# Schindler-EPFL-Lab/thermo-nerf

Hardware: AMD Instinct MI355X
Metric: rays/sec (forward-only render) @ 800x800, 192 samples/ray (higher is better)
Workload: dtype f32; 1 GPU; BASELINE metric configuration (configs[2]'s 192 samples/ray on the 800x800 frame of configs[1]): synthetic 800x800 RGB+thermal scene, P=(256,96)+192 samples/ray, chunk 640000, forward-only eval, scene weights; parallelism=ray-shard x1 (one frame per rank)

## Files before the change

### include/thermonerf_hip.h

```cpp
#ifndef THERMONERF_HIP_H
#define THERMONERF_HIP_H

#include <stddef.h>
#include <stdint.h>

#ifdef __cplusplus
extern "C" {
#endif

#define TN_OK 0
#define TN_ERR_NULL (-1)
#define TN_ERR_SHAPE (-2)
#define TN_ERR_UNSUPPORTED (-3)
#define TN_ERR_WORKSPACE (-4)
#define TN_ERR_LAUNCH (-5)

#define TN_MAX_LEVELS 16

typedef struct tn_hashgrid {
    const float *table;
    float scalings[TN_MAX_LEVELS];
    int32_t num_levels;
    int32_t log2_hashmap_size;
    const float *dense;
// ... 106 lines not shown
    float box_min[3], box_max[3];
    float thermal_lo, thermal_hi;
    float temperature_span, temperature_min;
    float to_world[12];
} tn_pointcloud_params;
int32_t tn_pointcloud_tile_rays(void);
int32_t tn_pointcloud_scan_width(void);
size_t tn_pointcloud_workspace_bytes(int64_t num_rays);
int tn_pointcloud_append(const float *origins, const float *directions, const float *depth, const float *accumulation,
                         const float *rgb, const float *thermal, int64_t num_rays, int64_t source_base,
                         const tn_pointcloud_params *params, const uint8_t *thermal_table, float *positions, uint8_t *colors,
                         float *temperature, uint8_t *thermal_colors, int64_t *source, int64_t capacity, int64_t *count,
                         void *workspace, size_t workspace_bytes, void *stream);

int32_t tn_knn_grid_resolution(int64_t num_points);
size_t tn_knn_workspace_bytes(int64_t num_points, int32_t grid_resolution);
int tn_knn(const float *positions, int64_t num_points, int32_t k, int32_t grid_resolution, int32_t *neighbor_index,
           float *neighbor_d2, double *mean_distance, void *workspace, size_t workspace_bytes, void *stream);
int tn_pointcloud_normals(const float *positions, const int32_t *neighbor_index, int64_t num_points, int32_t k,
                          const float *viewpoints, float *normals, void *stream);

typedef struct tn_mesh_params {
    float fx, fy, cx, cy;
    float w2c[12];
    float truncation, inv_truncation, min_accumulation;
    float lo[3], step[3];
    int32_t dims[3];
    float temperature_span, temperature_min;
    float to_world[12];
} tn_mesh_params;
int32_t tn_mesh_tile(void);
int32_t tn_mesh_scan_width(void);
size_t tn_mesh_workspace_bytes(int32_t nx, int32_t ny, int32_t nz);
int tn_tsdf_integrate(const float *depth, const float *accumulation, const float *thermal, const float *rgb, int32_t height,
                      int32_t width, const tn_mesh_params *params, float *volume, void *stream);
int tn_mesh_extract(const float *volume, const tn_mesh_params *params, const uint8_t *thermal_table, float *positions,
                    uint8_t *colors, float *temperature, uint8_t *thermal_colors, int64_t capacity_vertices, int32_t *triangles,
                    int64_t capacity_triangles, int64_t *counts, void *workspace, size_t workspace_bytes, void *stream);

size_t tn_mesh_components_workspace_bytes(int64_t num_vertices, int64_t num_triangles);
int tn_mesh_components(const int32_t *triangles, int64_t num_triangles, int64_t num_vertices, int32_t *labels,
                       int32_t *component_triangles, int64_t *summary, void *stream);
int tn_mesh_filter_components(const int32_t *triangles, int64_t num_triangles, int64_t num_vertices, const int32_t *labels,
                              const int32_t *component_triangles, const int64_t *summary, int64_t min_triangles,
                              int32_t largest_only, int32_t *vertex_source, int64_t capacity_vertices, int32_t *triangles_out,
                              int64_t capacity_triangles, int64_t *counts, void *workspace, size_t workspace_bytes, void *stream);

size_t tn_mesh_incidence_workspace_bytes(int64_t num_vertices, int64_t num_triangles);
int tn_mesh_incidence(const int32_t *triangles, int64_t num_triangles, int64_t num_vertices, int32_t *offsets, int32_t *corners,
                      void *workspace, size_t workspace_bytes, void *stream);
int tn_mesh_vertex_normals(const float *positions, const int32_t *triangles, int64_t num_triangles, int64_t num_vertices,
                           const int32_t *offsets, const int32_t *corners, float *normals, void *stream);
int tn_mesh_smooth(const float *positions_in, const int32_t *triangles, int64_t num_triangles, int64_t num_vertices,
                   const int32_t *offsets, const int32_t *corners, int32_t iterations, float lambda, float mu, float *positions_out,
                   float *scratch, void *stream);

int32_t tn_sort_tile(void);
size_t tn_sort_pairs_workspace_bytes(int64_t n);
int tn_sort_pairs(const uint64_t *keys_in, const int32_t *values_in, int64_t n, int key_bits, uint64_t *keys_out,
                  int32_t *values_out, void *workspace, size_t workspace_bytes, void *stream);

typedef struct tn_voxel_params {
    float origin[3];
    float voxel_size;
    int32_t dims[3];
} tn_voxel_params;
size_t tn_voxel_downsample_workspace_bytes(int64_t num_points);
int tn_voxel_downsample(const float *positions, const uint8_t *colors, const float *temperature, const uint8_t *thermal_colors,
                        const int64_t *source, int64_t num_points, const tn_voxel_params *params, float *positions_out,
                        uint8_t *colors_out, float *temperature_out, uint8_t *thermal_colors_out, int64_t *source_out,
                        int32_t *voxel_count, int64_t capacity, int64_t *count, void *workspace, size_t workspace_bytes, void *stream);


typedef struct tn_render_config {
    int32_t num_proposal_samples[2];
    int32_t num_nerf_samples;
    int32_t training;
    float pdf_anneal;
    float early_stop_transmittance;
    int32_t kernel_family;
    int32_t initial_sampler;
    int32_t sample_split;
    int32_t per_sample_jitter;
} tn_render_config;

typedef struct tn_render_inputs {
    const float *origins;
    const float *directions;
    const float *nears;
    const float *fars;
    const int32_t *camera_indices;
    const float *lin_bins0;
    const float *u1;
    const float *u2;
    const float *jitter;
} tn_render_inputs;

typedef struct tn_render_outputs {
    float *rgb;
    float *accumulation;
    float *depth;
    float *expected_depth;
    float *prop_depth_0;
    float *prop_depth_1;
    float *thermal;
    float *weights[3];
    float *spacing_bins[3];
    float *eucl_bins[3];
} tn_render_outputs;

size_t tn_render_workspace_bytes(const tn_render_config *cfg, int64_t num_rays);

int tn_render_rays_fwd(const tn_density_field *prop0, const tn_density_field *prop1, const tn_thermal_field *field,
                       const tn_render_config *cfg, const tn_render_inputs *in, const tn_render_outputs *out,
                       int64_t num_rays, void *workspace, size_t workspace_bytes, void *stream);

int tn_proposal_sample_fwd(const tn_density_field *prop0, const tn_density_field *prop1, const tn_render_config *cfg,
                           const tn_render_inputs *in, const tn_render_outputs *out, int64_t num_rays, void *workspace,
                           size_t workspace_bytes, void *stream);
int tn_field_render_fwd(const tn_thermal_field *field, const tn_render_config *cfg, const tn_render_inputs *in,
                        const tn_render_outputs *out, int64_t num_rays, void *workspace, size_t workspace_bytes,
                        void *stream);

int64_t tn_depth_bound_slots(int64_t first_ray, int64_t num_rays, int64_t chunk_rays);

int32_t tn_render_kernel_form(const tn_thermal_field *field, const tn_render_config *cfg, int64_t num_rays, int32_t pass);
int32_t tn_render_sample_split(const tn_thermal_field *field, const tn_render_config *cfg, int64_t num_rays);
int tn_field_render_chunked_fwd(const tn_thermal_field *field, const tn_render_config *cfg, const tn_render_inputs *in,
                                const tn_render_outputs *out, int64_t num_rays, void *workspace, size_t workspace_bytes,
                                int64_t first_ray, int64_t chunk_rays, float *depth_bounds, int32_t clip, void *stream);
int tn_expected_depth_clip_chunked(float *expected_depth, int64_t num_rays, int64_t first_ray, int64_t chunk_rays,
                                   const float *depth_bounds, void *stream);


size_t tn_hashgrid_prepare_bytes(const tn_hashgrid *grid, int64_t max_bytes);
int tn_hashgrid_prepare(const tn_hashgrid *grid_in, tn_hashgrid *grid_out, void *dense_dev, size_t dense_bytes,
                        void *stream);

size_t tn_field_prepare_bytes(const tn_thermal_field *field);
int tn_field_prepare(const tn_thermal_field *field, void *prepared_dev, size_t bytes, void *stream);

size_t tn_field_prepare_f16x3_bytes(const tn_thermal_field *field);
int tn_field_prepare_f16x3(const tn_thermal_field *field, void *prepared_dev, size_t bytes, void *stream);
size_t tn_field_prepare_bf16x6_bytes(const tn_thermal_field *field);
int tn_field_prepare_bf16x6(const tn_thermal_field *field, void *prepared_dev, size_t bytes, void *stream);

int tn_bf16x6_split_product(const float *a, const float *b, int64_t n, float *pieces_a, float *pieces_b, float *out, void *stream);
int tn_bf16_mfma_value_probe(float a_value, float b_value, float *out, void *stream);


#define TN_ACT_NONE 0
#define TN_ACT_RELU 1
#define TN_ACT_SIGMOID 2

int tn_hash_encode_fwd(const tn_hashgrid *grid, const tn_space *space, const float *positions, int64_t n, float *enc,
                       float *selector, void *stream);
int tn_hash_encode_bwd(const tn_hashgrid *grid, const tn_space *space, const float *positions, const float *d_enc,
                       int64_t n, float *d_table, void *stream);

int tn_hash_encode_bwd_levels(const tn_hashgrid *grid, const tn_space *space, const float *positions, const float *d_enc,
                              int64_t n, float *d_table, int32_t level_begin, int32_t level_end, void *stream);
size_t tn_hash_encode_bwd_spread_workspace_bytes(const tn_hashgrid *grid);
int tn_hash_encode_bwd_spread(const tn_hashgrid *grid, const tn_space *space, const float *positions, const float *d_enc,
                              int64_t n, float *d_table, int32_t level_begin, int32_t level_end, void *workspace,
                              size_t workspace_bytes, void *stream);

size_t tn_hash_encode_bwd_sorted_workspace_bytes(const tn_hashgrid *grid, int64_t n, int32_t level_begin);
int tn_hash_encode_bwd_sorted_first_level(const tn_hashgrid *grid, int64_t n);
int tn_hash_encode_bwd_sorted(const tn_hashgrid *grid, const tn_space *space, const float *positions, const float *d_enc,
                              int64_t n, float *d_table, int32_t level_begin, void *workspace, size_t workspace_bytes,
                              void *stream);

int tn_hash_encode_bwd_input(const tn_hashgrid *grid, const tn_space *space, const float *positions, const float *d_enc,
                             int64_t n, float *d_positions, void *stream);
int tn_frustum_positions_bwd(const float *d_positions, const float *starts, const float *ends, int64_t num_rays, int32_t n,
                             float *d_origins, float *d_directions, void *stream);

int tn_linear_fwd(const float *x, int32_t ldx, const tn_linear *lin, int32_t act, int64_t n, float *y, int32_t ldy,
                  void *stream);
size_t tn_linear_bwd_workspace_bytes(void);
int tn_linear_bwd(const float *x, int32_t ldx, const float *y, const float *dy, int32_t ldy, const tn_linear *lin,
                  int32_t act, int64_t n, float *dx, int32_t lddx, int32_t accumulate_dx, float *d_weight,
                  float *d_bias, void *workspace, size_t workspace_bytes, void *stream);

int tn_density_act_fwd(const float *raw, int32_t ld_raw, const float *selector, float average_init_density, int64_t n,
                       float *density, void *stream);
int tn_density_act_bwd(const float *raw, int32_t ld_raw, const float *selector, float average_init_density,
                       float trunc_exp_min, const float *d_density, int64_t n, float *d_raw, int32_t ld_d_raw,
                       int32_t clear_cols, void *stream);

int tn_weights_bwd(const float *deltas, const float *densities, const float *d_weights, int64_t num_rays, int32_t n,
                   float *d_densities, void *stream);

typedef struct tn_chain_layer {
    tn_linear lin;
    const float *x;
    int32_t ldx;
    int32_t act_x;
    float *d_weight;
    float *d_bias;
} tn_chain_layer;
size_t tn_linear_chain_bwd_workspace_bytes(void);
int tn_linear_chain_bwd(const tn_chain_layer *layers, int32_t num_layers, const float *y_top, int32_t act_top, const float *dy,
                        int32_t lddy, int64_t n, float *dx, int32_t lddx, int32_t accumulate_dx, void *workspace,
                        size_t workspace_bytes, void *stream);

int tn_field_fwd_taped(const tn_thermal_field *field, const float *positions, const float *directions,
                       const int32_t *camera_indices, int64_t num_rays, int32_t n, float *enc, float *selector, float *h1,
                       float *bo, float *density, float *c1, float *c2, float *rgb, float *t1, float *t2, float *thermal,
                       void *stream);
// ... 152 lines not shown
```

### thermo_nerf_amd/_hip.py

```python
from __future__ import annotations

import ctypes as C
import os
from typing import Optional

import torch

_LIB_NAME = "libthermonerf_hip.so"
_LIB_PATH = os.environ.get("THERMONERF_HIP_LIB") or os.path.join(os.path.dirname(os.path.abspath(__file__)), _LIB_NAME)

TN_MAX_LEVELS = 16

TN_OK = 0
_ERRORS = {
    -1: "TN_ERR_NULL: a required pointer is NULL",
    -2: "TN_ERR_SHAPE: a dimension is out of the supported range",
    -3: "TN_ERR_UNSUPPORTED: configuration not implemented by the kernels",
    -4: "TN_ERR_WORKSPACE: workspace too small",
    -5: "TN_ERR_LAUNCH: HIP reported a launch error",
}

_f32p = C.POINTER(C.c_float)
_i32p = C.POINTER(C.c_int32)

# ... 27 lines not shown
                ("one_minus_beta2", C.c_float), ("eps", C.c_float), ("weight_decay", C.c_float)]


ADAM_MAX_TENSORS = 32

class tn_field_grads(C.Structure):
    _fields_ = [(k, C.c_void_p) for k in ("base0_w", "base0_b", "base1_w", "base1_b", "head0_w", "head1_w", "head1_b", "head2_w",
                                         "head2_b", "th0_w", "th0_b", "th1_w", "th1_b", "thead_w", "thead_b")]


class tn_space(C.Structure):
    _fields_ = [
        ("contraction", C.c_int32),
        ("aabb_min", C.c_float * 3),
        ("aabb_max", C.c_float * 3),
        ("_pad", C.c_int32),
    ]


class tn_pointcloud_params(C.Structure):
    _fields_ = [("min_accumulation", C.c_float), ("box_min", C.c_float * 3), ("box_max", C.c_float * 3), ("thermal_lo", C.c_float),
                ("thermal_hi", C.c_float), ("temperature_span", C.c_float), ("temperature_min", C.c_float),
                ("to_world", C.c_float * 12)]


class tn_voxel_params(C.Structure):
    _fields_ = [("origin", C.c_float * 3), ("voxel_size", C.c_float), ("dims", C.c_int32 * 3)]


class tn_mesh_params(C.Structure):
    _fields_ = [("fx", C.c_float), ("fy", C.c_float), ("cx", C.c_float), ("cy", C.c_float), ("w2c", C.c_float * 12),
                ("truncation", C.c_float), ("inv_truncation", C.c_float), ("min_accumulation", C.c_float), ("lo", C.c_float * 3),
                ("step", C.c_float * 3), ("dims", C.c_int32 * 3), ("temperature_span", C.c_float), ("temperature_min", C.c_float),
                ("to_world", C.c_float * 12)]


class tn_density_field(C.Structure):
    _fields_ = [
        ("grid", tn_hashgrid),
        ("l0", tn_linear),
        ("l1", tn_linear),
        ("space", tn_space),
        ("average_init_density", C.c_float),
        ("_pad", C.c_int32),
    ]


class tn_thermal_field(C.Structure):
    _fields_ = [
        ("grid", tn_hashgrid),
        ("base0", tn_linear),
        ("base1", tn_linear),
        ("head0", tn_linear),
        ("head1", tn_linear),
        ("head2", tn_linear),
        ("th0", tn_linear),
        ("th1", tn_linear),
        ("thead", tn_linear),
        ("appearance", C.c_void_p),
        ("num_images", C.c_int32),
        ("app_dim", C.c_int32),
        ("geo_feat_dim", C.c_int32),
        ("use_average_appearance", C.c_int32),
        ("sh_shifted", C.c_int32),
        ("space", tn_space),
        ("average_init_density", C.c_float),
        ("prepared", C.c_void_p),
        ("prepared_f16x3", C.c_void_p),
        ("prepared_bf16x6", C.c_void_p),
    ]


class tn_render_config(C.Structure):
    _fields_ = [
        ("num_proposal_samples", C.c_int32 * 2),
        ("num_nerf_samples", C.c_int32),
        ("training", C.c_int32),
        ("pdf_anneal", C.c_float),
        ("early_stop_transmittance", C.c_float),
        ("kernel_family", C.c_int32),
        ("initial_sampler", C.c_int32),
        ("sample_split", C.c_int32),
        ("per_sample_jitter", C.c_int32),
    ]


class tn_render_inputs(C.Structure):
    _fields_ = [
        ("origins", C.c_void_p),
        ("directions", C.c_void_p),
        ("nears", C.c_void_p),
        ("fars", C.c_void_p),
        ("camera_indices", C.c_void_p),
        ("lin_bins0", C.c_void_p),
        ("u1", C.c_void_p),
        ("u2", C.c_void_p),
        ("jitter", C.c_void_p),
    ]


class tn_render_outputs(C.Structure):
    _fields_ = [
        ("rgb", C.c_void_p),
        ("accumulation", C.c_void_p),
        ("depth", C.c_void_p),
        ("expected_depth", C.c_void_p),
        ("prop_depth_0", C.c_void_p),
        ("prop_depth_1", C.c_void_p),
        ("thermal", C.c_void_p),
        ("weights", C.c_void_p * 3),
        ("spacing_bins", C.c_void_p * 3),
        ("eucl_bins", C.c_void_p * 3),
    ]


_fp = C.c_void_p


class tn_train_step(C.Structure):
    _fields_ = [("prop0", C.POINTER(tn_density_field)), ("prop1", C.POINTER(tn_density_field)),
                ("field_raw", C.POINTER(tn_thermal_field)), ("field", C.POINTER(tn_thermal_field)), ("prepared_bytes", C.c_size_t),
                ("cfg", C.POINTER(tn_render_config)), ("inputs", C.POINTER(tn_render_inputs)), ("num_rays", C.c_int64),
                ("spacing", _fp * 3), ("eucl", _fp * 3), ("weights", _fp * 3), ("prop_depth", _fp * 2),
                ("positions", _fp), ("starts", _fp), ("ends", _fp), ("deltas", _fp), ("ray_bias", _fp),
                ("enc", _fp), ("selector", _fp), ("density", _fp), ("rgb_samples", _fp), ("thermal_samples", _fp), ("base_out", _fp),
                ("jacobian", _fp),
                ("rgb", _fp), ("thermal", _fp), ("accumulation", _fp), ("depth", _fp), ("expected_depth", _fp), ("depth_scratch", _fp),
                ("workspace", _fp), ("workspace_bytes", C.c_size_t), ("zero_buffer", _fp), ("zero_bytes", C.c_size_t),
                ("distortion_mult", C.c_float), ("interlevel_mult", C.c_float),
                ("distortion_loss_pair", _fp), ("distortion_grad", _fp), ("interlevel_loss", _fp), ("interlevel_grad", _fp * 2),
                ("stream", _fp), ("second", _fp), ("third", _fp), ("wait_events", C.POINTER(C.c_void_p)), ("num_wait_events", C.c_int32)]


class tn_train_step_bwd_args(C.Structure):
    _fields_ = [("field", C.POINTER(tn_thermal_field)), ("num_rays", C.c_int64), ("n", C.c_int32)] + [
        (k, _fp) for k in ("positions", "starts", "ends", "deltas", "ray_bias", "enc", "selector", "density", "rgb_samples",
                           "thermal_samples", "base_out", "jacobian", "accumulation", "directions", "camera_indices",
                           "d_rgb", "d_thermal", "d_accumulation", "d_weights")] + [
        ("use_gradient_scaling", C.c_int32), ("pass_thermal_gradients", C.c_int32), ("split_form", C.c_int32),
        ("sh_direction_gradient", C.c_int32), ("trunc_exp_min", C.c_float)] + [
        (k, _fp) for k in ("d_rgb_samples", "d_thermal_samples", "d_density", "d_enc", "d_positions", "d_ray_sum", "d_ray_inputs")] + [
        ("grads", C.POINTER(tn_field_grads)), ("d_table", _fp), ("d_appearance", _fp), ("d_head0_bias", _fp), ("d_origins", _fp),
        ("d_directions", _fp), ("fused_workspace", _fp), ("fused_workspace_bytes", C.c_size_t), ("first_sorted_level", C.c_int32),
        ("sorted_workspace", _fp), ("sorted_workspace_bytes", C.c_size_t), ("spread", C.c_int32), ("spread_workspace", _fp),
        ("spread_workspace_bytes", C.c_size_t), ("overlap", C.c_int32), ("defer", C.c_int32), ("wait_second_first", C.c_int32),
        ("stream", _fp), ("second", _fp), ("third", _fp)]


_vp, _i64, _i32, _sz = C.c_void_p, C.c_int64, C.c_int32, C.c_size_t
SIGNATURES = {
    "tn_generate_rays": (C.c_int, [C.POINTER(C.c_float), C.c_float, C.c_float, C.c_float, C.c_float, _i32, _i32,
                                   C.POINTER(C.c_float), _i64, _i64, _vp, _vp, _vp, _vp]),
    "tn_frustum_positions": (C.c_int, [_vp, _vp, _vp, _vp, _i64, _i32, _vp, _vp]),
    "tn_frustum_from_edges": (C.c_int, [_vp, _vp, _vp, _i64, _i32, _vp, _vp, _vp, _vp, _vp]),
    "tn_density_fwd": (C.c_int, [C.POINTER(tn_density_field), _vp, _i64, _vp, _vp]),
    "tn_field_density_fwd": (C.c_int, [C.POINTER(tn_thermal_field), _vp, _i64, _vp, _vp, _vp]),
    "tn_field_heads_fwd": (C.c_int, [C.POINTER(tn_thermal_field), _vp, _vp, _vp, _i64, _i32, _vp, _vp, _vp]),
    "tn_camera_opt_fwd": (C.c_int, [_vp, _vp, _vp, _vp, _i64, _i32, _vp, _vp, _vp]),
    "tn_camera_opt_bwd": (C.c_int, [_vp, _vp, _vp, _vp, _vp, _i64, _i32, _vp, _vp, _vp]),
    "tn_sample_initial": (C.c_int, [_vp, _vp, _vp, _vp, _i64, _i32, _i32, _vp, _vp, _vp]),
    "tn_weights_fwd": (C.c_int, [_vp, _vp, _i64, _i32, _vp, _vp]),
    "tn_sample_pdf": (C.c_int, [_vp, _vp, _vp, _vp, _vp, _vp, _i64, _i32, _i32, _i32, _vp, _vp, _vp]),
    "tn_composite_fwd": (C.c_int, [_vp, _vp, _i64, _i32, _i32, _i32, _vp, _vp]),
    "tn_depth_fwd": (C.c_int, [_vp, _vp, _vp, _i64, _i32, _vp, _vp, _vp, _vp, _vp]),
    "tn_ssim_workspace_bytes": (_sz, [_i32, _i32, _i32]),
    "tn_ssim_fwd": (C.c_int, [_vp, _vp, _i32, _i32, _i32, C.c_float, _vp, _sz, _vp, _vp]),
    "tn_frame_to_rgb8": (C.c_int, [_vp, _i64, _i32, _i32, _vp, _vp, _vp, _vp, _vp]),
    "tn_otsu_thresholds": (C.c_int, [_vp, C.POINTER(C.c_int64), _i32, _vp, _vp, _vp]),
    "tn_pointcloud_tile_rays": (_i32, []),
    "tn_pointcloud_scan_width": (_i32, []),
    "tn_pointcloud_workspace_bytes": (_sz, [_i64]),
    "tn_pointcloud_append": (C.c_int, [_vp] * 6 + [_i64, _i64, C.POINTER(tn_pointcloud_params)] + [_vp] * 6 + [_i64, _vp, _vp, _sz, _vp]),
    "tn_knn_grid_resolution": (_i32, [_i64]),
    "tn_knn_workspace_bytes": (_sz, [_i64, _i32]),
    "tn_knn": (C.c_int, [_vp, _i64, _i32, _i32, _vp, _vp, _vp, _vp, _sz, _vp]),
    "tn_pointcloud_normals": (C.c_int, [_vp, _vp, _i64, _i32, _vp, _vp, _vp]),
    "tn_sort_tile": (_i32, []),
    "tn_sort_pairs_workspace_bytes": (_sz, [_i64]),
    "tn_sort_pairs": (C.c_int, [_vp, _vp, _i64, C.c_int, _vp, _vp, _vp, _sz, _vp]),
    "tn_voxel_downsample_workspace_bytes": (_sz, [_i64]),
    "tn_voxel_downsample": (C.c_int, [_vp] * 5 + [_i64, C.POINTER(tn_voxel_params)] + [_vp] * 6 + [_i64, _vp, _vp, _sz, _vp]),
    "tn_mesh_tile": (_i32, []),
    "tn_mesh_scan_width": (_i32, []),
    "tn_mesh_workspace_bytes": (_sz, [_i32, _i32, _i32]),
    "tn_tsdf_integrate": (C.c_int, [_vp] * 4 + [_i32, _i32, C.POINTER(tn_mesh_params), _vp, _vp]),
    "tn_mesh_extract": (C.c_int, [_vp, C.POINTER(tn_mesh_params)] + [_vp] * 5 + [_i64, _vp, _i64, _vp, _vp, _sz, _vp]),
    "tn_mesh_components_workspace_bytes": (_sz, [_i64, _i64]),
    "tn_mesh_components": (C.c_int, [_vp, _i64, _i64, _vp, _vp, _vp, _vp]),
    "tn_mesh_filter_components": (C.c_int, [_vp, _i64, _i64, _vp, _vp, _vp, _i64, _i32, _vp, _i64, _vp, _i64, _vp, _vp, _sz, _vp]),
    "tn_mesh_incidence_workspace_bytes": (_sz, [_i64, _i64]),
    "tn_mesh_incidence": (C.c_int, [_vp, _i64, _i64, _vp, _vp, _vp, _sz, _vp]),
    "tn_mesh_vertex_normals": (C.c_int, [_vp, _vp, _i64, _i64, _vp, _vp, _vp, _vp]),
    "tn_mesh_smooth": (C.c_int, [_vp, _vp, _i64, _i64, _vp, _vp, _i32, C.c_float, C.c_float, _vp, _vp, _vp]),
    "tn_render_workspace_bytes": (_sz, [C.POINTER(tn_render_config), _i64]),
    "tn_render_rays_fwd": (
        C.c_int,
        [C.POINTER(tn_density_field), C.POINTER(tn_density_field), C.POINTER(tn_thermal_field),
         C.POINTER(tn_render_config), C.POINTER(tn_render_inputs), C.POINTER(tn_render_outputs), _i64, _vp, _sz, _vp],
    ),
    "tn_proposal_sample_fwd": (
        C.c_int,
        [C.POINTER(tn_density_field), C.POINTER(tn_density_field), C.POINTER(tn_render_config),
         C.POINTER(tn_render_inputs), C.POINTER(tn_render_outputs), _i64, _vp, _sz, _vp],
    ),
    "tn_field_render_fwd": (
        C.c_int,
        [C.POINTER(tn_thermal_field), C.POINTER(tn_render_config), C.POINTER(tn_render_inputs),
         C.POINTER(tn_render_outputs), _i64, _vp, _sz, _vp],
    ),
    "tn_bf16x6_split_product": (C.c_int, [_vp, _vp, _i64, _vp, _vp, _vp, _vp]),
    "tn_bf16_mfma_value_probe": (C.c_int, [C.c_float, C.c_float, _vp, _vp]),
    "tn_depth_bound_slots": (_i64, [_i64, _i64, _i64]),
    "tn_render_kernel_form": (C.c_int32, [C.POINTER(tn_thermal_field), C.POINTER(tn_render_config), _i64, C.c_int32]),
    "tn_render_sample_split": (C.c_int32, [C.POINTER(tn_thermal_field), C.POINTER(tn_render_config), _i64]),
    "tn_field_render_chunked_fwd": (
        C.c_int,
        [C.POINTER(tn_thermal_field), C.POINTER(tn_render_config), C.POINTER(tn_render_inputs),
         C.POINTER(tn_render_outputs), _i64, _vp, _sz, _i64, _i64, _vp, _i32, _vp],
    ),
    "tn_expected_depth_clip_chunked": (C.c_int, [_vp, _i64, _i64, _i64, _vp, _vp]),
    "tn_hashgrid_prepare_bytes": (_sz, [C.POINTER(tn_hashgrid), _i64]),
    "tn_hashgrid_prepare": (C.c_int, [C.POINTER(tn_hashgrid), C.POINTER(tn_hashgrid), _vp, _sz, _vp]),
    "tn_field_prepare_bytes": (_sz, [C.POINTER(tn_thermal_field)]),
    "tn_field_prepare": (C.c_int, [C.POINTER(tn_thermal_field), _vp, _sz, _vp]),
    "tn_field_prepare_f16x3_bytes": (_sz, [C.POINTER(tn_thermal_field)]),
    "tn_field_prepare_f16x3": (C.c_int, [C.POINTER(tn_thermal_field), _vp, _sz, _vp]),
    "tn_field_prepare_bf16x6_bytes": (_sz, [C.POINTER(tn_thermal_field)]),
    "tn_field_prepare_bf16x6": (C.c_int, [C.POINTER(tn_thermal_field), _vp, _sz, _vp]),
    "tn_hash_encode_fwd": (C.c_int, [C.POINTER(tn_hashgrid), C.POINTER(tn_space), _vp, _i64, _vp, _vp, _vp]),
    "tn_hash_encode_bwd": (C.c_int, [C.POINTER(tn_hashgrid), C.POINTER(tn_space), _vp, _vp, _i64, _vp, _vp]),
    "tn_hash_encode_bwd_levels": (C.c_int, [C.POINTER(tn_hashgrid), C.POINTER(tn_space), _vp, _vp, _i64, _vp, _i32, _i32, _vp]),
    "tn_hash_encode_bwd_spread_workspace_bytes": (_sz, [C.POINTER(tn_hashgrid)]),
    "tn_hash_encode_bwd_spread": (C.c_int, [C.POINTER(tn_hashgrid), C.POINTER(tn_space), _vp, _vp, _i64, _vp, _i32, _i32, _vp, _sz, _vp]),
    "tn_hash_encode_bwd_sorted_workspace_bytes": (_sz, [C.POINTER(tn_hashgrid), _i64, _i32]),
    "tn_hash_encode_bwd_sorted_first_level": (C.c_int, [C.POINTER(tn_hashgrid), _i64]),
    "tn_hash_encode_bwd_sorted": (C.c_int, [C.POINTER(tn_hashgrid), C.POINTER(tn_space), _vp, _vp, _i64, _vp, _i32, _vp, _sz, _vp]),
    "tn_linear_fwd": (C.c_int, [_vp, _i32, C.POINTER(tn_linear), _i32, _i64, _vp, _i32, _vp]),
    "tn_linear_bwd_workspace_bytes": (_sz, []),
    "tn_linear_bwd": (C.c_int, [_vp, _i32, _vp, _vp, _i32, C.POINTER(tn_linear), _i32, _i64, _vp, _i32, _i32, _vp, _vp, _vp,
                                _sz, _vp]),
    "tn_density_act_fwd": (C.c_int, [_vp, _i32, _vp, C.c_float, _i64, _vp, _vp]),
    "tn_density_act_bwd": (C.c_int, [_vp, _i32, _vp, C.c_float, C.c_float, _vp, _i64, _vp, _i32, _i32, _vp]),
    "tn_weights_bwd": (C.c_int, [_vp, _vp, _vp, _i64, _i32, _vp, _vp]),
    "tn_gradient_scale_bwd": (C.c_int, [_vp, _vp, _i64, _vp, _vp, _vp, _vp]),
    "tn_linear_chain_bwd_workspace_bytes": (_sz, []),
    "tn_linear_chain_bwd": (C.c_int, [C.POINTER(tn_chain_layer), _i32, _vp, _i32, _vp, _i32, _i64, _vp, _i32, _i32, _vp, _sz, _vp]),
    "tn_field_fwd_taped": (C.c_int, [C.POINTER(tn_thermal_field), _vp, _vp, _vp, _i64, _i32] + [_vp] * 12),
    "tn_density_fwd_train": (C.c_int, [C.POINTER(tn_density_field), _vp, _i64, _vp, _vp, _vp, _vp, _vp]),
    "tn_density_bwd_train": (C.c_int, [C.POINTER(tn_density_field), _vp, _vp, _vp, _vp, _i64, C.c_float, _vp, _vp, _vp, _vp, _vp, _vp]),
    "tn_ray_head_fwd": (C.c_int, [C.POINTER(tn_thermal_field), _vp, _vp, _i64, _vp, _vp]),
    "tn_ray_head_bwd": (C.c_int, [C.POINTER(tn_thermal_field), _vp, _vp, _i64, _vp, _vp, _vp, _vp, _vp, _vp]),
    "tn_field_fwd_train": (C.c_int, [C.POINTER(tn_thermal_field), _vp, _vp, _i64, _i32] + [_vp] * 8),
    "tn_field_bwd_fused_workspace_bytes": (_sz, [_i64, _i32]),
    "tn_field_bwd_fused": (C.c_int, [C.POINTER(tn_thermal_field), _i64, _i32, _vp, _vp, _vp, _vp, _vp, _vp, _vp, _vp, _i32, C.c_float,
                                     _i32, _vp, _vp, _vp, _vp, _vp, C.POINTER(tn_field_grads), _vp, _sz, _vp]),
    "tn_composite_bwd": (C.c_int, [_vp, _vp, _vp, _vp, _i64, _i32, _i32, _vp, _vp, _vp]),
    "tn_color_input_fwd": (C.c_int, [C.POINTER(tn_thermal_field), _vp, _vp, _i32, _vp, _i32, _i64, _i32, _vp, _vp]),
    "tn_color_input_bwd": (C.c_int, [C.POINTER(tn_thermal_field), _vp, _vp, _i32, _i64, _i32, _vp, _i32, _vp, _vp, _vp, _vp]),
    "tn_hash_encode_bwd_input": (C.c_int, [C.POINTER(tn_hashgrid), C.POINTER(tn_space), _vp, _vp, _i64, _vp, _vp]),
    "tn_frustum_positions_bwd": (C.c_int, [_vp, _vp, _vp, _i64, _i32, _vp, _vp, _vp]),
    "tn_ray_render_fwd": (C.c_int, [_vp, _vp, _vp, _vp, _i64, _i32, _vp, _vp, _vp, _vp, _vp]),
    "tn_ray_render_bwd": (C.c_int, [_vp] * 11 + [_i64, _i32, _vp, _vp, _vp, _vp]),
    "tn_ray_render_depth_fwd": (C.c_int, [_vp] * 6 + [_i64, _i32] + [_vp] * 8),
    "tn_image_losses": (C.c_int, [_vp, _vp, _vp, _vp, _i64, _vp, _vp, _vp, _vp]),
    "tn_sum_scalars": (C.c_int, [C.POINTER(C.c_void_p), _i32, _vp, _vp]),
    "tn_distortion_loss": (C.c_int, [_vp, _vp, _i64, _i32, C.c_float, _vp, _vp, _vp]),
    "tn_distortion_loss_term": (C.c_int, [_vp, _vp, _i64, _i32, C.c_float, C.c_float, _vp, _vp, _vp]),
    "tn_interlevel_loss": (C.c_int, [_vp, _vp, _vp, _vp, _i64, _i32, _i32, C.c_float, _vp, _vp, _vp]),
    "tn_interlevel_loss_levels": (C.c_int, [_vp, _vp, _i64, _i32, _i32, C.POINTER(C.c_void_p), C.POINTER(C.c_void_p),
                                            C.POINTER(C.c_int32), C.c_float, _vp, C.POINTER(C.c_void_p), _vp]),
    "tn_adam_step": (C.c_int, [C.POINTER(tn_adam_tensor), _i32, _vp]),
    "tn_train_step_fwd": (C.c_int, [C.POINTER(tn_train_step)]),
    "tn_train_step_bwd": (C.c_int, [C.POINTER(tn_train_step_bwd_args)]),
    "tn_version": (C.c_char_p, []),
}

_lib: Optional[C.CDLL] = None


def lib_path() -> str:
    return _LIB_PATH


def load() -> C.CDLL:
    global _lib
    if _lib is not None:
        return _lib
    if not os.path.exists(_LIB_PATH):
        raise RuntimeError(
            f"{_LIB_NAME} not found at {_LIB_PATH}; build it with `python -c 'import __graft_entry__ as g; g.build()'` "
            "(or `make -C thermo_nerf_amd/csrc`). thermo_nerf_amd has no CPU/PyTorch fallback for its kernels."
        )
    try:
        lib = C.CDLL(_LIB_PATH)
    except OSError as e:
        raise RuntimeError(f"failed to load {_LIB_PATH}: {e}") from e
    for name, (restype, argtypes) in SIGNATURES.items():
# ... 188 lines not shown
```

### thermo_nerf_amd/csrc/tn_render.hip

```cpp
#include "tn_field_eval.h"

#include <type_traits>

#ifndef TN_PROP_WAVES
#define TN_PROP_WAVES 4
#endif
#ifndef TN_RESAMPLE_BLOCK
#define TN_RESAMPLE_BLOCK 16
#endif
#ifndef TN_PROP_SPLIT
#define TN_PROP_SPLIT 1
#endif
#ifndef TN_PDF_LOAD_PRIO
#define TN_PDF_LOAD_PRIO 1
#endif
#ifndef TN_PROP_GATHER_PRIO
#define TN_PROP_GATHER_PRIO 1
#endif
using namespace tn;

namespace tn {
int launch_main_mfma(const tn_thermal_field *field, const tn_render_config *cfg, const tn_render_inputs *in,
                     const tn_render_outputs *out, long long num_rays, const float *spacing_ws, DepthSlots minmax,
                     hipStream_t stream, int split, float *seg_scratch);
int launch_main_b6(const tn_thermal_field *field, const tn_render_config *cfg, const tn_render_inputs *in,
                   const tn_render_outputs *out, long long num_rays, const float *spacing_ws, DepthSlots minmax,
                   hipStream_t stream);
int launch_main_h3(const tn_thermal_field *field, const tn_render_config *cfg, const tn_render_inputs *in,
                   const tn_render_outputs *out, long long num_rays, const float *spacing_ws, DepthSlots minmax,
                   hipStream_t stream);
}

namespace {

constexpr int kBlock = 256;
constexpr int kWaves = kBlock / TN_WAVE;
constexpr int PH = 16;
constexpr size_t kWsMid = 2048;
constexpr int kPropWFloats = 208;

struct PropNet {
    Grid g;
    tn_space space;
    const float *w0, *b0, *w1, *b1;
    float avg;
};

struct PropArgs {
    PropNet net[2];
    const float *origins, *dirs, *nears, *fars;
    const float *lin0, *u1, *u2, *jitter;
    int jper;
    const float *wk;
    long long R;
    int P0, P1, S, training;
    int lin;
    float anneal;
    float *ws_spacing;
    float *out_spacing[3];
    float *out_eucl[3];
    float *out_w[2];
    float *prop_depth[2];
};

__device__ __forceinline__ float prop_level(const PropNet &net, const TwoLayerLds &w, float ox, float oy, float oz,
                                            float dx, float dy, float dz, float s_near, float s_far, bool lin,
                                            const float *bins, int n, float *wts, int lane) {
    const Space sp = make_space(net.space);
    for (int base = 0; base < n; base += 64) {
        const int i = base + lane;
        if (i < n) {
            const float st = spacing_to_eucl<true>(bins[i], s_near, s_far, lin);
            const float en = spacing_to_eucl<true>(bins[i + 1], s_near, s_far, lin);
            float px, py, pz;
            const float sel = normalize_position<true>(sp, frustum_pos(ox, dx, st, en), frustum_pos(oy, dy, st, en),
                                                 frustum_pos(oz, dz, st, en), px, py, pz);
            const float dens = (net.g.num_levels == 5)
                                   ? proposal_density_scalar<PH, 5, true>(net.g, as_scalar(net.w0), as_scalar(net.b0),
                                                                          as_scalar(net.w1), as_scalar(net.b1), net.avg, px, py, pz, sel)
                                   : proposal_density_eval<PH, 0, true>(net.g, w, net.avg, px, py, pz, sel);
            wts[i] = mul_rn(sub_rn(en, st), dens);
        }
    }
    float carry = 0.0f, carry_w = 0.0f;
    int med_idx = n;
    for (int base = 0; base < n; base += 64) {
        const int i = base + lane;
        const bool ok = i < n;
        const float dd = ok ? wts[i] : 0.0f;
        const float incl = wave_incl_scan(dd, lane);
        const float excl = carry + wave_excl_from_incl(incl, lane);
        const float wi = ok ? nan_to_num(mul_rn(sub_rn(1.0f, __expf(-dd)), __expf(-excl))) : 0.0f;
        carry += lane_value<63>(incl);
        const float incl_w = wave_incl_scan(wi, lane) + carry_w;
        const unsigned long long hit = __ballot(ok && (incl_w >= 0.5f));
        if (hit && med_idx == n) med_idx = base + __ffsll((long long)hit) - 1;
        carry_w = lane_value<63>(incl_w);
        if (ok) wts[i] = wi;
    }
    const int idx = min(med_idx, n - 1);
    const float st = spacing_to_eucl<true>(bins[idx], s_near, s_far, lin);
    const float en = spacing_to_eucl<true>(bins[idx + 1], s_near, s_far, lin);
    return add_rn(st, en) / 2.0f;
}

__device__ __forceinline__ void pdf_resample(const float *wts, const float *bins, int n_in, float *cdf,
                                             const float *u, bool jittered, const float *jrow, bool jper, float anneal, int n_out,
// ... 597 lines not shown
            wbl += mul_rn(wi, c[2]);
            wth += mul_rn(wi, th);
            wsteps += mul_rn(wi, step);
            if (a.out_w && ok) a.out_w[r * S + i] = wi;
            if (base + 64 >= S) {
                const int src = (S - 1) - base;
                last_r = __shfl(c[0], src, 64);
                last_g = __shfl(c[1], src, 64);
                last_b = __shfl(c[2], src, 64);
                last_t = __shfl(th, src, 64);
            }
        }
        wsum = wave_sum(wsum);
        wr = wave_sum(wr); wg = wave_sum(wg); wbl = wave_sum(wbl); wth = wave_sum(wth); wsteps = wave_sum(wsteps);
        const int idx = min(med_idx, S - 1);
        if (lane == 0) {
            const float bg = sub_rn(1.0f, wsum);
            float cr = add_rn(wr, mul_rn(last_r, bg)), cg = add_rn(wg, mul_rn(last_g, bg)), cb = add_rn(wbl, mul_rn(last_b, bg));
            float ct = add_rn(wth, mul_rn(last_t, bg));
            if (!a.training) {
                cr = fminf(fmaxf(cr, 0.0f), 1.0f); cg = fminf(fmaxf(cg, 0.0f), 1.0f); cb = fminf(fmaxf(cb, 0.0f), 1.0f);
                ct = fminf(fmaxf(ct, 0.0f), 1.0f);
            }
            a.rgb[r * 3 + 0] = cr; a.rgb[r * 3 + 1] = cg; a.rgb[r * 3 + 2] = cb;
            a.thermal[r] = ct;
            a.acc[r] = wsum;
            const float st = spacing_to_eucl(sb[idx], s_near, s_far, lin), en = spacing_to_eucl(sb[idx + 1], s_near, s_far, lin);
            a.depth[r] = add_rn(st, en) / 2.0f;
            a.expected[r] = wsteps / add_rn(wsum, 1e-10f);
        }
    }
    depth_bounds_flush(a.minmax, mm_slot, smin, smax, lane);
}

__global__ void depth_clip_kernel(float *__restrict__ expected, long long num_rays, const unsigned *mm) {
    const long long r = (long long)blockIdx.x * blockDim.x + threadIdx.x;
    if (r >= num_rays) return;
    const float lo = key2f(mm[0]), hi = key2f(mm[1]);
    expected[r] = fminf(fmaxf(expected[r], lo), hi);
}

__global__ void depth_slots_init_kernel(unsigned *keys, int slots) {
    const int i = blockIdx.x * blockDim.x + threadIdx.x;
    if (i < slots) {
        keys[2 * i] = 0xffffffffu;
        keys[2 * i + 1] = 0u;
    }
}

__global__ void depth_slots_export_kernel(unsigned *keys, int slots) {
    const int i = blockIdx.x * blockDim.x + threadIdx.x;
    if (i < 2 * slots) keys[i] = __float_as_uint(key2f(keys[i]));
}

__global__ void depth_clip_chunked_kernel(float *__restrict__ expected, long long num_rays, long long first_ray, long long chunk_rays,
                                          const float *__restrict__ bounds) {
    const long long r = (long long)blockIdx.x * blockDim.x + threadIdx.x;
    if (r >= num_rays) return;
    const long long slot = (first_ray + r) / chunk_rays - first_ray / chunk_rays;
    expected[r] = fminf(fmaxf(expected[r], bounds[2 * slot]), bounds[2 * slot + 1]);
}

inline size_t align_up(size_t x, size_t a) { return (x + a - 1) / a * a; }

inline PropNet make_prop(const tn_density_field *f) {
    PropNet p;
    p.g = tn_make_grid(f->grid);
    p.space = f->space;
    p.w0 = f->l0.weight; p.b0 = f->l0.bias; p.w1 = f->l1.weight; p.b1 = f->l1.bias;
    p.avg = f->average_init_density;
    return p;
}

inline unsigned ray_grid(long long R, int blocks_per_cu) {
    const long long need = (R + kWaves - 1) / kWaves;
    const long long cap = 256LL * blocks_per_cu;
    return (unsigned)(need < cap ? (need < 1 ? 1 : need) : cap);
}

}

extern "C" {

size_t tn_render_workspace_bytes(const tn_render_config *cfg, int64_t num_rays) {
    if (!cfg || num_rays < 0) return 0;
    const size_t tiles = (size_t)((num_rays + 63) >> 6);
    const int P0 = cfg->num_proposal_samples[0], P1 = cfg->num_proposal_samples[1];
    const size_t nmax = (size_t)(P0 > P1 ? P0 : P1);
    return align_up(tn_ws_bin_floats(num_rays, cfg->num_nerf_samples) * sizeof(float), 256) + kWsMid +
           tiles * 64 * (nmax + (size_t)P1 + 1) * sizeof(float);
}

static int check_render_common(const tn_render_config *cfg, int64_t num_rays, void *workspace, size_t workspace_bytes) {
    if (!cfg || !workspace) return TN_ERR_NULL;
    const int P0 = cfg->num_proposal_samples[0], P1 = cfg->num_proposal_samples[1], S = cfg->num_nerf_samples;
    if (P0 < 1 || P1 < 1 || S < 1 || P0 > 1024 || P1 > 1024 || S > 1024 || num_rays < 0) return TN_ERR_SHAPE;
    if (cfg->initial_sampler != 0 && cfg->initial_sampler != 1) return TN_ERR_UNSUPPORTED;
    if (workspace_bytes < tn_render_workspace_bytes(cfg, num_rays)) return TN_ERR_WORKSPACE;
    return TN_OK;
}

static inline unsigned *ws_minmax(void *workspace, int64_t num_rays, int S) {
    return reinterpret_cast<unsigned *>(reinterpret_cast<char *>(workspace) +
                                        align_up(tn_ws_bin_floats(num_rays, S) * sizeof(float), 256));
}

int tn_proposal_sample_fwd(const tn_density_field *prop0, const tn_density_field *prop1, const tn_render_config *cfg,
                           const tn_render_inputs *in, const tn_render_outputs *out, int64_t num_rays, void *workspace,
                           size_t workspace_bytes, void *stream) {
    if (num_rays == 0) return TN_OK;
    if (!prop0 || !prop1 || !in || !out) return TN_ERR_NULL;
    TN_TRY(check_render_common(cfg, num_rays, workspace, workspace_bytes));
    if (!in->origins || !in->directions || !in->nears || !in->fars || !in->lin_bins0 || !in->u1 || !in->u2) return TN_ERR_NULL;
    if (cfg->training && !in->jitter) return TN_ERR_NULL;
    TN_TRY(tn_check_density_field(prop0));
    TN_TRY(tn_check_density_field(prop1));
    if (prop0->l0.out_dim != PH || prop1->l0.out_dim != PH) return TN_ERR_UNSUPPORTED;
    const int P0 = cfg->num_proposal_samples[0], P1 = cfg->num_proposal_samples[1], S = cfg->num_nerf_samples;
    hipStream_t s = (hipStream_t)stream;
    PropArgs pa;
    pa.net[0] = make_prop(prop0);
    pa.net[1] = make_prop(prop1);
    pa.origins = in->origins; pa.dirs = in->directions; pa.nears = in->nears; pa.fars = in->fars;
    pa.lin0 = in->lin_bins0; pa.u1 = in->u1; pa.u2 = in->u2;
    pa.jitter = cfg->training ? in->jitter : nullptr;
    pa.jper = cfg->per_sample_jitter != 0;
    pa.R = num_rays; pa.P0 = P0; pa.P1 = P1; pa.S = S; pa.training = cfg->training; pa.anneal = cfg->pdf_anneal;
    pa.lin = cfg->initial_sampler == 1;
    pa.ws_spacing = reinterpret_cast<float *>(workspace);
    for (int i = 0; i < 3; ++i) { pa.out_spacing[i] = out->spacing_bins[i]; pa.out_eucl[i] = out->eucl_bins[i]; }
    pa.out_w[0] = out->weights[0]; pa.out_w[1] = out->weights[1];
    pa.prop_depth[0] = out->prop_depth_0; pa.prop_depth[1] = out->prop_depth_1;
    const int nmax = P0 > P1 ? P0 : P1;
    int nbmax = nmax > S ? nmax : S;
    nbmax += 1;
    const size_t prop_smem = (size_t)(two_layer_floats(2 * prop0->grid.num_levels, PH, 1) +
                                      two_layer_floats(2 * prop1->grid.num_levels, PH, 1) +
                                      kWaves * (3 * nbmax + nmax)) * sizeof(float);

    {
        float *wk = reinterpret_cast<float *>(reinterpret_cast<char *>(workspace) +
                                              align_up(tn_ws_bin_floats(num_rays, S) * sizeof(float), 256) + 256);
        hipLaunchKernelGGL(prop_weights_kmajor_kernel, dim3(2), dim3(256), 0, s, pa.net[0], pa.net[1], wk,
                           ws_minmax(workspace, num_rays, S));
        pa.wk = wk;
    }
    const bool small_call = tn_render_kernel_form(nullptr, cfg, num_rays, 0) == 2;
    if (!small_call) {
        PropRaysArgs ra;
        ra.p = pa;
        ra.nmax = nmax;
        char *scratch = reinterpret_cast<char *>(workspace) + align_up(tn_ws_bin_floats(num_rays, S) * sizeof(float), 256) + kWsMid;
        const size_t tiles = (size_t)((num_rays + 63) >> 6);
        ra.w_scratch = reinterpret_cast<float *>(scratch);
        ra.b1_scratch = ra.w_scratch + tiles * 64 * (size_t)nmax;
        const size_t rsmem = (size_t)(two_layer_floats(2 * prop0->grid.num_levels, PH, 1) +
                                      two_layer_floats(2 * prop1->grid.num_levels, PH, 1) + (P0 + 1) + (P1 + 1) + (S + 1)) *
                             sizeof(float);
        const long long need = ((long long)tiles + kWaves - 1) / kWaves;
        constexpr long long kMaxGrid = 256LL * TN_PROP_WAVES;
        const unsigned grid = (unsigned)(need < kMaxGrid ? (need < 1 ? 1 : need) : kMaxGrid);
        const int nd0 = pa.net[0].g.num_dense, nd1 = pa.net[1].g.num_dense;
        const bool five = pa.net[0].g.num_levels == 5 && pa.net[1].g.num_levels == 5;
        bool lean = five && !pa.jitter && !pa.lin && pa.anneal == 1.0f && pa.net[0].space.contraction && pa.net[1].space.contraction &&
                    !pa.out_w[0] && !pa.out_w[1];
        for (int i = 0; i < 3; ++i) lean = lean && !pa.out_spacing[i] && !pa.out_eucl[i];
        constexpr long long kSlots = 256LL * TN_PROP_WAVES * kWaves;
        if (TN_PROP_SPLIT && lean && five && 4 * (long long)tiles < 3 * kSlots && ((nd0 == 5 && nd1 == 4) || (nd0 == 0 && nd1 == 0)) && P0 >= 64 &&
            P1 >= 32) {
            PropSplitArgs sa;
            sa.ra = ra;
            const int counts[2] = {P0, P1}, kcap[2] = {8, 4};
            for (int l = 0; l < 2; ++l) {
                long long k = (3 * kSlots + (long long)tiles - 1) / (long long)tiles;
                if (k > kcap[l]) k = kcap[l];
                if (k < 1) k = 1;
                sa.len[l] = (int)((counts[l] + k - 1) / k);
                sa.k[l] = (counts[l] + sa.len[l] - 1) / sa.len[l];
            }
            auto blocks = [&](long long units) {
                const long long nb = (units + kWaves - 1) / kWaves;
                return dim3((unsigned)(nb < kMaxGrid ? (nb < 1 ? 1 : nb) : kMaxGrid));
            };
            const size_t lds0 = (size_t)(P0 + 1) * sizeof(float);
            const size_t ldsr0 = (size_t)(P0 + 1 + P1 + 1) * sizeof(float), ldsr1 = (size_t)(P0 + 1 + S + 1) * sizeof(float);
            if (nd0 == 5) {
                hipLaunchKernelGGL((proposal_density_segments_kernel<5, 0>), blocks((long long)tiles * sa.k[0]), dim3(kBlock), lds0, s, sa);
                hipLaunchKernelGGL(proposal_resample_kernel<0>, blocks((long long)tiles), dim3(kBlock), ldsr0, s, sa);
                hipLaunchKernelGGL((proposal_density_segments_kernel<4, 1>), blocks((long long)tiles * sa.k[1]), dim3(kBlock), 0, s, sa);
            } else {
                hipLaunchKernelGGL((proposal_density_segments_kernel<0, 0>), blocks((long long)tiles * sa.k[0]), dim3(kBlock), lds0, s, sa);
                hipLaunchKernelGGL(proposal_resample_kernel<0>, blocks((long long)tiles), dim3(kBlock), ldsr0, s, sa);
                hipLaunchKernelGGL((proposal_density_segments_kernel<0, 1>), blocks((long long)tiles * sa.k[1]), dim3(kBlock), 0, s, sa);
            }
            hipLaunchKernelGGL(proposal_resample_kernel<1>, blocks((long long)tiles), dim3(kBlock), ldsr1, s, sa);
            TN_LAUNCH_CHECK();
            return TN_OK;
        }
        if (five && nd0 == 5 && nd1 == 4 && lean)
            hipLaunchKernelGGL((proposal_rays_kernel<5, 4, true>), dim3(grid), dim3(kBlock), rsmem, s, ra);
        else if (five && nd0 == 5 && nd1 == 4)
            hipLaunchKernelGGL((proposal_rays_kernel<5, 4, false>), dim3(grid), dim3(kBlock), rsmem, s, ra);
        else if (nd0 == 0 && nd1 == 0 && lean)
            hipLaunchKernelGGL((proposal_rays_kernel<0, 0, true>), dim3(grid), dim3(kBlock), rsmem, s, ra);
        else if (nd0 == 0 && nd1 == 0)
            hipLaunchKernelGGL((proposal_rays_kernel<0, 0, false>), dim3(grid), dim3(kBlock), rsmem, s, ra);
        else
            hipLaunchKernelGGL((proposal_rays_kernel<-1, -1, false>), dim3(grid), dim3(kBlock), rsmem, s, ra);
        TN_LAUNCH_CHECK();
        return TN_OK;
    }
    if (prop_smem > 64 * 1024 && !tn_ensure_dynamic_lds<proposal_kernel>(prop_smem)) return TN_ERR_LAUNCH;
    hipLaunchKernelGGL(proposal_kernel, dim3(ray_grid(num_rays, 8)), dim3(kBlock), prop_smem, s, pa, nmax, nbmax);
    TN_LAUNCH_CHECK();
    return TN_OK;
}

static int field_render_fwd(const tn_thermal_field *field, const tn_render_config *cfg, const tn_render_inputs *in,
                            const tn_render_outputs *out, int64_t num_rays, void *workspace, size_t workspace_bytes,
                            int64_t first_ray, int64_t chunk_rays, float *depth_bounds, int clip, void *stream) {
    if (num_rays == 0) return TN_OK;
    if (!field || !in || !out) return TN_ERR_NULL;
    TN_TRY(check_render_common(cfg, num_rays, workspace, workspace_bytes));
    if (!in->origins || !in->directions || !in->nears || !in->fars) return TN_ERR_NULL;
    if (!out->rgb || !out->accumulation || !out->depth || !out->expected_depth || !out->thermal) return TN_ERR_NULL;
    if (cfg->training && !in->camera_indices) return TN_ERR_NULL;
    TN_TRY(tn_check_thermal_field(field));
    if (field->geo_feat_dim != GF) return TN_ERR_UNSUPPORTED;
    const int S = cfg->num_nerf_samples;
    hipStream_t s = (hipStream_t)stream;
    const float *ws_spacing = reinterpret_cast<const float *>(workspace);
    DepthSlots minmax{ws_minmax(workspace, num_rays, S), 0, 0};
    int slots = 1;
    if (depth_bounds) {
        if (chunk_rays < 64 || chunk_rays % 64 != 0 || first_ray < 0 || first_ray % 64 != 0) return TN_ERR_UNSUPPORTED;
        const int64_t n_slots = (first_ray + num_rays - 1) / chunk_rays - first_ray / chunk_rays + 1;
        if (n_slots > (1 << 20)) return TN_ERR_SHAPE;
        slots = (int)n_slots;
        minmax = DepthSlots{reinterpret_cast<unsigned *>(depth_bounds), (long long)first_ray, (long long)chunk_rays};
        hipLaunchKernelGGL(depth_slots_init_kernel, dim3((slots + 255) / 256), dim3(256), 0, s, minmax.keys, slots);
    }
    const bool split_ok = !out->weights[2] && tn_render_kernel_form(field, cfg, num_rays, 1) == 1 &&
                          (field->prepared_bf16x6 || field->prepared_f16x3);
    if (field->prepared_bf16x6 && split_ok) {
        TN_TRY(launch_main_b6(field, cfg, in, out, (long long)num_rays, ws_spacing, minmax, s));
    } else if (field->prepared_f16x3 && split_ok) {
        TN_TRY(launch_main_h3(field, cfg, in, out, (long long)num_rays, ws_spacing, minmax, s));
    } else if (field->prepared) {
        const int split = out->weights[2] ? 1 : tn_render_sample_split(field, cfg, num_rays);
        float *seg_scratch = reinterpret_cast<float *>(reinterpret_cast<char *>(workspace) +
                                                       align_up(tn_ws_bin_floats(num_rays, S) * sizeof(float), 256) + kWsMid);
        TN_TRY(launch_main_mfma(field, cfg, in, out, (long long)num_rays, ws_spacing, minmax, s, split, seg_scratch));
    } else {
        MainArgs ma;
        ma.g = tn_make_grid(field->grid);
        ma.space = field->space;
        ma.b0w = field->base0.weight; ma.b0b = field->base0.bias; ma.b1w = field->base1.weight; ma.b1b = field->base1.bias;
        ma.heads = make_heads_args(field);
        ma.avg = field->average_init_density;
        ma.origins = in->origins; ma.dirs = in->directions; ma.nears = in->nears; ma.fars = in->fars;
        ma.cam = in->camera_indices;
        ma.spacing = ws_spacing;
        ma.R = num_rays; ma.S = S; ma.training = cfg->training; ma.lin = cfg->initial_sampler == 1;
        ma.rgb = out->rgb; ma.acc = out->accumulation; ma.depth = out->depth; ma.expected = out->expected_depth;
        ma.thermal = out->thermal; ma.out_w = out->weights[2]; ma.minmax = minmax;
        const size_t main_smem = (size_t)(two_layer_floats(2 * field->grid.num_levels, HW, 1 + GF) +
                                          heads_floats(GF, field->app_dim)) * sizeof(float);
        if (!tn_ensure_dynamic_lds<main_valu_kernel>(main_smem)) return TN_ERR_LAUNCH;
        hipLaunchKernelGGL(main_valu_kernel, dim3(ray_grid(num_rays, 2)), dim3(kBlock), main_smem, s, ma);
        TN_LAUNCH_CHECK();
    }
    if (depth_bounds) {
        hipLaunchKernelGGL(depth_slots_export_kernel, dim3((2 * slots + 255) / 256), dim3(256), 0, s, minmax.keys, slots);
        if (clip)
            hipLaunchKernelGGL(depth_clip_chunked_kernel, dim3((unsigned)((num_rays + 255) / 256)), dim3(256), 0, s,
                               out->expected_depth, (long long)num_rays, (long long)first_ray, (long long)chunk_rays, depth_bounds);
    } else {
        hipLaunchKernelGGL(depth_clip_kernel, dim3((unsigned)((num_rays + 255) / 256)), dim3(256), 0, s, out->expected_depth,
                           (long long)num_rays, minmax.keys);
    }
    TN_LAUNCH_CHECK();
    return TN_OK;
}

int tn_field_render_fwd(const tn_thermal_field *field, const tn_render_config *cfg, const tn_render_inputs *in,
                        const tn_render_outputs *out, int64_t num_rays, void *workspace, size_t workspace_bytes,
                        void *stream) {
    return field_render_fwd(field, cfg, in, out, num_rays, workspace, workspace_bytes, 0, 0, nullptr, 1, stream);
}

static int sample_split_kmax(const tn_thermal_field *field, const tn_render_config *cfg) {
    if (!cfg || !field || cfg->sample_split == 1) return 1;
    if (cfg->training || cfg->early_stop_transmittance > 0.0f || !field->prepared || field->prepared_bf16x6 || field->prepared_f16x3) return 1;
    const int S = cfg->num_nerf_samples, P0 = cfg->num_proposal_samples[0], P1 = cfg->num_proposal_samples[1];
    const int scratch = (P0 > P1 ? P0 : P1) + P1 + 1;
    int kmax = (scratch - S) / 12;
    if (kmax > S / 8) kmax = S / 8;
    if (kmax > 8) kmax = 8;
    return kmax < 2 ? 1 : kmax;
}

int32_t tn_render_kernel_form(const tn_thermal_field *field, const tn_render_config *cfg, int64_t num_rays, int32_t pass) {
    if (!cfg) return 0;
    if (cfg->kernel_family == 1 || cfg->kernel_family == 2) return cfg->kernel_family;
    if (pass == 0) return num_rays < (cfg->training ? 65536 : 24576) ? 2 : 1;
    const bool split_precision = field && !cfg->training && (field->prepared_bf16x6 || field->prepared_f16x3);
    const int64_t from = split_precision ? 40960 : (sample_split_kmax(field, cfg) >= 2 ? 8192 : 57344);
    return num_rays < from ? 2 : 1;
}

int32_t tn_render_sample_split(const tn_thermal_field *field, const tn_render_config *cfg, int64_t num_rays) {
    if (!cfg || !field || num_rays <= 0) return 1;
    const int kmax = sample_split_kmax(field, cfg);
    if (kmax < 2 || tn_render_kernel_form(field, cfg, num_rays, 1) != 1) return 1;
    const int S = cfg->num_nerf_samples;
    if (cfg->sample_split > 1) return cfg->sample_split < kmax ? cfg->sample_split : kmax;
    const long long slots = 2048, tiles = (num_rays + 63) / 64;
    if (tiles >= 4 * slots) return 1;
    long long cost[9], best_cost = 0;
    for (int k = 1; k <= kmax; ++k) {
        cost[k] = ((tiles * k + slots - 1) / slots) * (2 * ((S + k - 1) / k) + 1);
        if (k == 1 || cost[k] < best_cost) best_cost = cost[k];
    }
    int best = 1;
    for (int k = 2; k <= kmax; ++k)
        if (100 * cost[k] <= 107 * best_cost) best = k;
    return best;
}

int64_t tn_depth_bound_slots(int64_t first_ray, int64_t num_rays, int64_t chunk_rays) {
    if (num_rays <= 0 || chunk_rays <= 0 || first_ray < 0) return 0;
    return (first_ray + num_rays - 1) / chunk_rays - first_ray / chunk_rays + 1;
}

int tn_field_render_chunked_fwd(const tn_thermal_field *field, const tn_render_config *cfg, const tn_render_inputs *in,
                                const tn_render_outputs *out, int64_t num_rays, void *workspace, size_t workspace_bytes,
                                int64_t first_ray, int64_t chunk_rays, float *depth_bounds, int32_t clip, void *stream) {
    if (!depth_bounds) return TN_ERR_NULL;
    return field_render_fwd(field, cfg, in, out, num_rays, workspace, workspace_bytes, first_ray, chunk_rays, depth_bounds,
                            clip, stream);
}

int tn_expected_depth_clip_chunked(float *expected_depth, int64_t num_rays, int64_t first_ray, int64_t chunk_rays,
                                   const float *depth_bounds, void *stream) {
    if (num_rays == 0) return TN_OK;
    if (!expected_depth || !depth_bounds) return TN_ERR_NULL;
    if (num_rays < 0 || chunk_rays < 1 || first_ray < 0) return TN_ERR_SHAPE;
    hipLaunchKernelGGL(depth_clip_chunked_kernel, dim3((unsigned)((num_rays + 255) / 256)), dim3(256), 0, (hipStream_t)stream,
                       expected_depth, (long long)num_rays, (long long)first_ray, (long long)chunk_rays, depth_bounds);
    TN_LAUNCH_CHECK();
    return TN_OK;
}

int tn_render_rays_fwd(const tn_density_field *prop0, const tn_density_field *prop1, const tn_thermal_field *field,
                       const tn_render_config *cfg, const tn_render_inputs *in, const tn_render_outputs *out,
                       int64_t num_rays, void *workspace, size_t workspace_bytes, void *stream) {
    TN_TRY(tn_proposal_sample_fwd(prop0, prop1, cfg, in, out, num_rays, workspace, workspace_bytes, stream));
    return tn_field_render_fwd(field, cfg, in, out, num_rays, workspace, workspace_bytes, stream);
}

const char *tn_version(void) { return "thermonerf_hip 0.1 gfx950"; }

}
```

### thermo_nerf_amd/csrc/tn_render_mfma.hip

```cpp
#include "tn_field_eval.h"
#ifndef TN_MFMA_MLP_PRIO
#define TN_MFMA_MLP_PRIO 1
#endif
#ifndef TN_MFMA_THERMAL_PRIO
#define TN_MFMA_THERMAL_PRIO (TN_MFMA_MLP_PRIO ? TN_MFMA_MLP_PRIO + 1 : 0)
#endif
#ifndef TN_EVAL_GATHER_PRIO
#define TN_EVAL_GATHER_PRIO 0
#endif
#ifndef TN_TRAIN_GATHER_PRIO
#define TN_TRAIN_GATHER_PRIO 1
#endif

#ifndef TN_BASE2_STAGED
#define TN_BASE2_STAGED 1
#endif
#ifndef TN_T2_PRESCALE
#define TN_T2_PRESCALE 1
#endif

using namespace tn;

namespace {

// ... 435 lines not shown
            }
        }
        wsum = wave_sum(wsum);
        wr = wave_sum(wr); wg = wave_sum(wg); wbl = wave_sum(wbl); wth = wave_sum(wth); wsteps = wave_sum(wsteps);
        const int idx = min(med_idx, S - 1);
        if (lane == 0) {
            const float bg = sub_rn(1.0f, wsum);
            float c0 = add_rn(wr, mul_rn(last_r, bg)), c1 = add_rn(wg, mul_rn(last_g, bg)), c2 = add_rn(wbl, mul_rn(last_b, bg));
            float ct = add_rn(wth, mul_rn(last_t, bg));
            if (!a.training) {
                c0 = fminf(fmaxf(c0, 0.0f), 1.0f); c1 = fminf(fmaxf(c1, 0.0f), 1.0f); c2 = fminf(fmaxf(c2, 0.0f), 1.0f);
                ct = fminf(fmaxf(ct, 0.0f), 1.0f);
            }
            a.rgb[r * 3 + 0] = c0; a.rgb[r * 3 + 1] = c1; a.rgb[r * 3 + 2] = c2;
            a.thermal[r] = ct;
            a.acc[r] = wsum;
            const float st = spacing_to_eucl<true>(sb[idx], s_near, s_far, lin), en = spacing_to_eucl<true>(sb[idx + 1], s_near, s_far, lin);
            a.depth[r] = add_rn(st, en) / 2.0f;
            a.expected[r] = wsteps / add_rn(wsum, 1e-10f);
        }
        __builtin_amdgcn_fence(__ATOMIC_RELEASE, "wavefront");
        __builtin_amdgcn_wave_barrier();
        __builtin_amdgcn_fence(__ATOMIC_ACQUIRE, "wavefront");
    }
    depth_bounds_flush(a.minmax, mm_slot, smin, smax, lane);
}

__device__ __forceinline__ float fast_sigmoid(float x) {
    return __builtin_amdgcn_rcpf(1.0f + __expf(-x));
}

__device__ __forceinline__ float fast_sigmoid_prescaled(float x) {
    return __builtin_amdgcn_rcpf(1.0f + __builtin_amdgcn_exp2f(x));
}

template <int ACT>
__device__ __forceinline__ float2 out_dot_fast(const float *wrow, int h, const f32x16 (&x)[2][2]) {
    float p0 = 0.0f, p1 = 0.0f;
#pragma unroll
    for (int mt = 0; mt < 2; ++mt) {
#pragma unroll
        for (int q = 0; q < 4; ++q) {
            const float4 w = *reinterpret_cast<const float4 *>(wrow + 32 * mt + 8 * q + 4 * h);
            const float ww[4] = {w.x, w.y, w.z, w.w};
#pragma unroll
            for (int e = 0; e < 4; ++e) {
                const float a0 = x[mt][0][4 * q + e], a1 = x[mt][1][4 * q + e];
                const float v0 = ACT == 2 ? fast_sigmoid_prescaled(a0) : ACT ? fast_sigmoid(a0) : relu_bits(a0);
                const float v1 = ACT == 2 ? fast_sigmoid_prescaled(a1) : ACT ? fast_sigmoid(a1) : relu_bits(a1);
                p0 = fmaf(ww[e], v0, p0);
                p1 = fmaf(ww[e], v1, p1);
            }
        }
    }
    return make_float2(p0, p1);
}

__device__ __forceinline__ f32x16 c0_frag(const float4 *p) {
    f32x16 v;
#pragma unroll
    for (int q = 0; q < 4; ++q) {
        const float4 t = p[q * 64];
        v[4 * q] = t.x; v[4 * q + 1] = t.y; v[4 * q + 2] = t.z; v[4 * q + 3] = t.w;
    }
    return v;
}

#ifndef TN_FIELD_STAMPS
#define TN_FIELD_STAMPS 0
#endif
#if TN_FIELD_STAMPS
constexpr int kStampBlocks = 16, kStampSamples = 192, kStampSlots = 16;
__device__ unsigned int tn_field_stamp_buf[kStampBlocks * 2 * kStampSamples * kStampSlots];
#define TN_STAMP(k)                                            \
    do {                                                       \
        __builtin_amdgcn_sched_barrier(0);                     \
        stamp[k] = (unsigned int)__builtin_amdgcn_s_memtime(); \
        __builtin_amdgcn_sched_barrier(0);                     \
    } while (0)
#else
#define TN_STAMP(k) do { } while (0)
#endif

template <bool DENSE, bool SPLIT = false>
__global__ void __launch_bounds__(kRaysBlock, 1) main_mfma_rays_kernel(MfmaArgs a) {
    extern __shared__ __attribute__((aligned(16))) float lds[];
    {
        const float4 *src = reinterpret_cast<const float4 *>(a.blob);
        float4 *dst = reinterpret_cast<float4 *>(lds);
        for (int i = threadIdx.x; i < RAYS_BLOB_FLOATS / 4; i += kRaysBlock) {
            float4 v = src[i < OFF_W_SH / 4 ? i : i + (OFF_W3 - OFF_W_SH) / 4];
#if TN_T2_PRESCALE
            if ((i >= A_T2 * 16 && i < A_SH * 16) || (i >= OFF_B_T2 / 4 && i < OFF_B_T2 / 4 + 16)) {
                const float k = -1.44269504088896341f;
                v = make_float4(mul_rn(v.x, k), mul_rn(v.y, k), mul_rn(v.z, k), mul_rn(v.w, k));
            }
#endif
            dst[i] = v;
        }
    }
    __syncthreads();
    const float *A = lds + OFF_A;
    const Space sp = make_space(a.space);
    const int lane = threadIdx.x & 63, wave = threadIdx.x >> 6, h = lane >> 5;
    const bool lin = a.lin != 0;
    const int S = a.S;
    float4 *c0s = reinterpret_cast<float4 *>(lds + RAYS_OFF_C0) + wave * RAYS_C0_SLOTS * 64 + lane;
    const long long groups = (a.R + 63) >> 6;
    const long long stride = (long long)gridDim.x * kRaysWaves;
    const int K = SPLIT ? a.split : 1;
    const long long vgroups = groups * K;
    float smin = INFINITY, smax = -INFINITY;
    long long mm_slot = 0;
#if TN_FIELD_STAMPS
    unsigned int stamp[kStampSlots] = {};
    int tile_no = -1;
#endif
    for (long long vg = (long long)blockIdx.x * kRaysWaves + wave; vg < vgroups; vg += stride) {
#if TN_FIELD_STAMPS
        ++tile_no;
#endif
        const long long grp = SPLIT ? vg / K : vg;
        const int s0 = SPLIT ? (int)(vg - grp * K) * a.seg_len : 0;
        const int s1 = SPLIT ? (s0 + a.seg_len < S ? s0 + a.seg_len : S) : S;
        if (a.minmax.chunk_rays > 0 && a.minmax.slot(grp * 64) != mm_slot) {
            depth_bounds_flush(a.minmax, mm_slot, smin, smax, lane);
            mm_slot = a.minmax.slot(grp * 64);
        }
        const long long r = grp * 64 + lane;
        const bool live = r < a.R;
        const long long rc = live ? r : a.R - 1;
        const float ox = a.origins[rc * 3], oy = a.origins[rc * 3 + 1], oz = a.origins[rc * 3 + 2];
        const float dx = a.dirs[rc * 3], dy = a.dirs[rc * 3 + 1], dz = a.dirs[rc * 3 + 2];
        const float s_near = spacing_fn(a.nears[rc], lin), s_far = spacing_fn(a.fars[rc], lin);
        const float *tb = a.spacing + tn_ws_bin(grp * 64, 0, S) + (rc - grp * 64);
        f32x16 c00;
        {
            f32x16 c0[2][2];
            float sx = dx, sy = dy, sz = dz;
            if (a.sh_shifted) {
                sx = add_rn(sx, 1.0f) / 2.0f; sy = add_rn(sy, 1.0f) / 2.0f; sz = add_rn(sz, 1.0f) / 2.0f;
            }
            float c[16];
            sh16(sx, sy, sz, c);
#pragma unroll
            for (int mt = 0; mt < 2; ++mt) {
                c0[mt][0] = bias_frag(lds + OFF_B_C1_EVAL, mt, h);
                c0[mt][1] = c0[mt][0];
            }
#pragma unroll
            for (int s = 0; s < 8; ++s) {
                float bs0, bs1;
                swap32(c[2 * s], c[2 * s + 1], bs0, bs1);
#pragma unroll
                for (int mt = 0; mt < 2; ++mt) {
                    const float aw = A[(A_SH + mt * 8 + s) * 64 + lane];
                    MFMA32(c0[mt][0], aw, bs0);
                    MFMA32(c0[mt][1], aw, bs1);
                }
            }
            c00 = c0[0][0];
#pragma unroll
            for (int q = 0; q < 4; ++q) {
                c0s[(0 + q) * 64] = make_float4(c0[0][1][4 * q], c0[0][1][4 * q + 1], c0[0][1][4 * q + 2], c0[0][1][4 * q + 3]);
                c0s[(4 + q) * 64] = make_float4(c0[1][0][4 * q], c0[1][0][4 * q + 1], c0[1][0][4 * q + 2], c0[1][0][4 * q + 3]);
                c0s[(8 + q) * 64] = make_float4(c0[1][1][4 * q], c0[1][1][4 * q + 1], c0[1][1][4 * q + 2], c0[1][1][4 * q + 3]);
            }
        }
        float en = spacing_to_eucl<true>(tb[(size_t)s0 * 64], s_near, s_far, lin);
        float accum = 0.0f, cum_w = 0.0f;
        float wsum = 0.0f, wr = 0.0f, wg = 0.0f, wbl = 0.0f, wth = 0.0f, wsteps = 0.0f;
        float cr = 0.0f, cg = 0.0f, cb = 0.0f, th = 0.0f, med = 0.0f, step = 0.0f;
        bool med_found = false;
        float sb_next = tb[(size_t)(s0 + 1) * 64];
        for (int i = s0; i < s1; ++i) {
            TN_STAMP(0);
            const float st = en;
            en = spacing_to_eucl<true>(sb_next, s_near, s_far, lin);
            sb_next = tb[(size_t)(i + 2 <= S ? i + 2 : S) * 64];
            step = add_rn(st, en) / 2.0f;
            float px, py, pz;
            const float sel = normalize_position<true>(sp, frustum_pos(ox, dx, st, en), frustum_pos(oy, dy, st, en),
                                                 frustum_pos(oz, dz, st, en), px, py, pz);
            float bt0[16], bt1[16];
#if TN_FIELD_STAMPS
            hash_encode_pipelined_raw<L16, LG, DENSE ? kFieldDense : 0, TN_EVAL_GATHER_PRIO>(
                a.g, px, py, pz, [&](int l, const HashTaps &t, const float2 (&fc)[8]) {
                    if (l % LG == 0) TN_STAMP(1 + 2 * (l / LG));
                    const float2 f = hash_blend(t, fc);
                    if (l % LG == 0) TN_STAMP(2 + 2 * (l / LG));
                    swap32(f.x, f.y, bt0[l], bt1[l]);
                });
            TN_STAMP(9);
#else
            hash_encode_pipelined<L16, LG, DENSE ? kFieldDense : 0, TN_EVAL_GATHER_PRIO>(a.g, px, py, pz,
                                                                    [&](int l, float2 f) { swap32(f.x, f.y, bt0[l], bt1[l]); });
#endif
#if TN_MFMA_MLP_PRIO
            __builtin_amdgcn_s_setprio(TN_MFMA_MLP_PRIO);
#endif
            f32x16 h1[2][2];
#pragma unroll
            for (int mt = 0; mt < 2; ++mt) {
                h1[mt][0] = bias_frag(lds + OFF_B_BASE1, mt, h);
                h1[mt][1] = h1[mt][0];
            }
#pragma unroll
            for (int s = 0; s < 16; ++s) {
#pragma unroll
                for (int mt = 0; mt < 2; ++mt) {
                    const float aw = A[(A_BASE1 + mt * 16 + s) * 64 + lane];
                    MFMA32(h1[mt][0], aw, bt0[s]);
                    MFMA32(h1[mt][1], aw, bt1[s]);
                }
            }
            float g[2][8];
            base2_geo<TN_BASE2_STAGED != 0>(A, lds + OFF_B_BASE2, lane, h1, g);
            float raw, unused;
            swap32(g[0][0], g[1][0], raw, unused);
            const float dens = mul_rn(mul_rn(a.avg, __expf(raw)), sel);
            TN_STAMP(10);
            {
                f32x16 x1[2][2] = {{c00, c0_frag(c0s)}, {c0_frag(c0s + 4 * 64), c0_frag(c0s + 8 * 64)}}, x2[2][2];
#pragma unroll
                for (int s = 0; s < 8; ++s) {
#pragma unroll
                    for (int mt = 0; mt < 2; ++mt) {
                        const float aw = A[(A_C1 + mt * 8 + s) * 64 + lane];
                        MFMA32(x1[mt][0], aw, g[0][s]);
                        MFMA32(x1[mt][1], aw, g[1][s]);
                    }
                }
                layer64(A, A_C2, lds + OFF_B_C2, lane, h, x1, x2);
                TN_STAMP(11);
                const float *w3 = lds + RAYS_OFF_W3;
                cr = fast_sigmoid(combine_halves(out_dot_fast<0>(w3, h, x2)) + w3[192]);
                cg = fast_sigmoid(combine_halves(out_dot_fast<0>(w3 + 64, h, x2)) + w3[193]);
                cb = fast_sigmoid(combine_halves(out_dot_fast<0>(w3 + 128, h, x2)) + w3[194]);
                TN_STAMP(12);
            }
#if TN_MFMA_THERMAL_PRIO != TN_MFMA_MLP_PRIO
            __builtin_amdgcn_s_setprio(TN_MFMA_THERMAL_PRIO);
#endif
            {
                f32x16 x1[2][2], x2[2][2];
                layer_geo(A, A_T1, lds + OFF_B_T1, lane, h, g, x1);
                layer64(A, A_T2, lds + OFF_B_T2, lane, h, x1, x2);
                TN_STAMP(13);
                const float *wt = lds + RAYS_OFF_WTH;
                th = combine_halves(out_dot_fast<TN_T2_PRESCALE ? 2 : 1>(wt, h, x2)) + wt[64];
                TN_STAMP(14);
            }
#if TN_MFMA_MLP_PRIO
            __builtin_amdgcn_s_setprio(0);
#endif
            cr = nan_to_num(cr); cg = nan_to_num(cg); cb = nan_to_num(cb); th = nan_to_num(th);
            const float dd = mul_rn(sub_rn(en, st), dens);
            const float wi = nan_to_num(mul_rn(sub_rn(1.0f, __expf(-dd)), __expf(-accum)));
            accum += dd;
            cum_w += wi;
            if (!med_found && cum_w >= 0.5f) {
                med_found = true;
                med = step;
            }
            wsum += wi;
            wr += mul_rn(wi, cr);
            wg += mul_rn(wi, cg);
            wbl += mul_rn(wi, cb);
            wth += mul_rn(wi, th);
            wsteps += mul_rn(wi, step);
            smin = fminf(smin, step);
            smax = fmaxf(smax, step);
#if TN_FIELD_STAMPS
            TN_STAMP(15);
            if (blockIdx.x < kStampBlocks && (wave & 3) == 0 && tile_no == 1 && i < kStampSamples && lane < kStampSlots) {
                unsigned int v = stamp[0];
#pragma unroll
                for (int k = 1; k < kStampSlots; ++k) v = lane == k ? stamp[k] : v;
                tn_field_stamp_buf[((blockIdx.x * 2 + (wave >> 2)) * kStampSamples + i) * kStampSlots + lane] = v;
            }
#endif
            if (SPLIT) {
                a.seg_cum[((size_t)grp * S + i) * 64 + lane] = cum_w;
                continue;
            }
            if (a.out_w && live) a.out_w[r * S + i] = wi;
            if (a.early_eps > 0.0f && i + 1 < S && __all(__expf(-accum) < a.early_eps)) {
                const float e0 = spacing_to_eucl<true>(tb[(size_t)(S - 1) * 64], s_near, s_far, lin);
                const float e1 = spacing_to_eucl<true>(tb[(size_t)S * 64], s_near, s_far, lin);
                smax = fmaxf(smax, add_rn(e0, e1) / 2.0f);
                break;
            }
        }
        if (SPLIT) {
            float *rec = a.seg_rec + (size_t)vg * SEG_ROWS * 64 + lane;
            const float row[SEG_ROWS] = {accum, wsum, wr, wg, wbl, wth, wsteps, cr, cg, cb, th, step};
#pragma unroll
            for (int k = 0; k < SEG_ROWS; ++k) rec[k * 64] = row[k];
            continue;
        }
        if (live) {
            const float bg = sub_rn(1.0f, wsum);
            const float c0 = add_rn(wr, mul_rn(cr, bg)), c1 = add_rn(wg, mul_rn(cg, bg)), c2 = add_rn(wbl, mul_rn(cb, bg));
            const float ct = add_rn(wth, mul_rn(th, bg));
            a.rgb[r * 3 + 0] = fminf(fmaxf(c0, 0.0f), 1.0f);
            a.rgb[r * 3 + 1] = fminf(fmaxf(c1, 0.0f), 1.0f);
            a.rgb[r * 3 + 2] = fminf(fmaxf(c2, 0.0f), 1.0f);
            a.thermal[r] = fminf(fmaxf(ct, 0.0f), 1.0f);
            a.acc[r] = wsum;
            a.depth[r] = med_found ? med : step;
            a.expected[r] = wsteps / add_rn(wsum, 1e-10f);
        }
    }
    depth_bounds_flush(a.minmax, mm_slot, smin, smax, lane);
}

__global__ void segments_combine_kernel(MfmaArgs a) {
    const long long r = (long long)blockIdx.x * blockDim.x + threadIdx.x;
    if (r >= a.R) return;
    const long long grp = r >> 6;
    const int lane = (int)(r & 63), S = a.S, K = a.split;
    const bool lin = a.lin != 0;
    float depth_so_far = 0.0f;
    float wsum = 0.0f, wr = 0.0f, wg = 0.0f, wbl = 0.0f, wth = 0.0f, wsteps = 0.0f, med = 0.0f;
    bool med_found = false;
    const float *rec = a.seg_rec + (size_t)grp * K * SEG_ROWS * 64 + lane;
    for (int j = 0; j < K; ++j, rec += SEG_ROWS * 64) {
        float T = __expf(-depth_so_far);
        T = T == T ? T : 0.0f;
        const float total = add_rn(wsum, mul_rn(T, rec[1 * 64]));
        if (!med_found && total >= 0.5f) {
            const int s0 = j * a.seg_len, s1 = s0 + a.seg_len < S ? s0 + a.seg_len : S;
            const float *cum = a.seg_cum + ((size_t)grp * S + s0) * 64 + lane;
            int i = s0;
            for (; i < s1 - 1; ++i, cum += 64)
                if (add_rn(wsum, mul_rn(T, cum[0])) >= 0.5f) break;
            const float s_near = spacing_fn(a.nears[r], lin), s_far = spacing_fn(a.fars[r], lin);
            const float *tb = a.spacing + tn_ws_bin(grp * 64, 0, S) + lane;
            med = add_rn(spacing_to_eucl<true>(tb[(size_t)i * 64], s_near, s_far, lin),
                         spacing_to_eucl<true>(tb[(size_t)(i + 1) * 64], s_near, s_far, lin)) / 2.0f;
            med_found = true;
        }
        wsum = total;
        wr = add_rn(wr, mul_rn(T, rec[2 * 64]));
        wg = add_rn(wg, mul_rn(T, rec[3 * 64]));
        wbl = add_rn(wbl, mul_rn(T, rec[4 * 64]));
        wth = add_rn(wth, mul_rn(T, rec[5 * 64]));
        wsteps = add_rn(wsteps, mul_rn(T, rec[6 * 64]));
        depth_so_far += rec[0];
    }
    rec -= SEG_ROWS * 64;
    const float cr = rec[7 * 64], cg = rec[8 * 64], cb = rec[9 * 64], th = rec[10 * 64], step = rec[11 * 64];
    const float bg = sub_rn(1.0f, wsum);
    const float c0 = add_rn(wr, mul_rn(cr, bg)), c1 = add_rn(wg, mul_rn(cg, bg)), c2 = add_rn(wbl, mul_rn(cb, bg));
    const float ct = add_rn(wth, mul_rn(th, bg));
    a.rgb[r * 3 + 0] = fminf(fmaxf(c0, 0.0f), 1.0f);
    a.rgb[r * 3 + 1] = fminf(fmaxf(c1, 0.0f), 1.0f);
    a.rgb[r * 3 + 2] = fminf(fmaxf(c2, 0.0f), 1.0f);
    a.thermal[r] = fminf(fmaxf(ct, 0.0f), 1.0f);
    a.acc[r] = wsum;
    a.depth[r] = med_found ? med : step;
    a.expected[r] = wsteps / add_rn(wsum, 1e-10f);
}


struct TapedArgs {
    Grid g;
    tn_space space;
    const float *blob;
    const float *appearance;
    float avg;
    int sh_shifted;
    const float *positions;
    const float *dirs;
    const int *cam;
    long long N;
    int n;
    float *enc, *sel, *h1, *bo, *density, *c1, *c2, *rgb, *t1, *t2, *thermal;
    const float *ray_bias;
    float *jac;
};

template <int ACT>
__device__ __forceinline__ void tape_store(float *dst, long long row0, long long N, int lane, int h, f32x16 (&x)[2][2]) {
#pragma unroll
    for (int mt = 0; mt < 2; ++mt) {
#pragma unroll
        for (int nt = 0; nt < 2; ++nt) {
            const long long row = row0 + 32 * nt + (lane & 31);
#pragma unroll
            for (int q = 0; q < 4; ++q) {
                float4 v;
                float *pv = &v.x;
#pragma unroll
                for (int e = 0; e < 4; ++e) {
                    const float a = x[mt][nt][4 * q + e];
                    const float y = ACT == 1 ? relu_bits(a) : sigmoidf(a);
                    x[mt][nt][4 * q + e] = y;
                    pv[e] = y;
                }
                if (row < N) *reinterpret_cast<float4 *>(dst + row * 64 + 32 * mt + 8 * q + 4 * h) = v;
            }
        }
    }
}

#ifndef TN_TRAIN_JAC_LG
#define TN_TRAIN_JAC_LG 2
#endif
template <bool TAPE, bool JAC = false>
__global__ void __launch_bounds__(kBlock, 2) field_fwd_taped_kernel(TapedArgs a) {
    extern __shared__ __attribute__((aligned(16))) float lds[];
    {
        const float4 *src = reinterpret_cast<const float4 *>(a.blob);
        float4 *dst = reinterpret_cast<float4 *>(lds);
        for (int i = threadIdx.x; i < BLOB_FLOATS / 4; i += kBlock) dst[i] = src[i];
    }
    __syncthreads();
    const float *A = lds + OFF_A;
    const Space sp = make_space(a.space);
    const int lane = threadIdx.x & 63, wave = threadIdx.x >> 6, h = lane >> 5;
    const long long passes = (a.N + 63) >> 6;
    const long long stride = (long long)gridDim.x * kWaves;
    for (long long ps = (long long)blockIdx.x * kWaves + wave; ps < passes; ps += stride) {
        const long long row0 = ps * 64;
        const long long i = row0 + lane;
        const bool live = i < a.N;
        const long long ic = live ? i : a.N - 1;
        const long long ray = ic / a.n;
        float px, py, pz;
        const float sel = normalize_position(sp, a.positions[ic * 3], a.positions[ic * 3 + 1], a.positions[ic * 3 + 2], px, py, pz);
        float bt0[16], bt1[16];
        if (!TAPE) {
            float2 *et = reinterpret_cast<float2 *>(a.enc) + ps * (16 * 64) + lane;
            if (JAC) {
                float2 *jt = reinterpret_cast<float2 *>(a.jac) + ps * (16 * 3 * 64) + lane;
                hash_encode_pipelined_raw<L16, TN_TRAIN_JAC_LG, 0, TN_TRAIN_GATHER_PRIO>(a.g, px, py, pz, [&](int l, const HashTaps &t, const float2 (&fc)[8]) {
                    float2 jc[3];
                    const float2 f = hash_blend_jac(t, fc, jc);
                    const float s = a.g.scal[l];
                    et[l * 64] = f;
#pragma unroll
                    for (int c = 0; c < 3; ++c) jt[(l * 3 + c) * 64] = make_float2(jc[c].x * s, jc[c].y * s);
                    swap32(f.x, f.y, bt0[l], bt1[l]);
                });
            } else {
                hash_encode_pipelined<L16, LG, 0, TN_TRAIN_GATHER_PRIO>(a.g, px, py, pz, [&](int l, float2 f) {
// ... 88 lines not shown
                    }
                }
            } else {
#pragma unroll
                for (int nt = 0; nt < 2; ++nt) {
                    long long smp = row0 + 32 * nt + (lane & 31);
                    if (smp >= a.N) smp = a.N - 1;
                    const float *rb = a.ray_bias + (smp / a.n) * 64;
#pragma unroll
                    for (int mt = 0; mt < 2; ++mt) x1[mt][nt] = bias_frag(rb, mt, h);
                }
#pragma unroll
                for (int s = 0; s < 8; ++s) {
#pragma unroll
                    for (int mt = 0; mt < 2; ++mt) {
                        const float aw = A[(A_C1 + mt * 8 + s) * 64 + lane];
                        MFMA32(x1[mt][0], aw, g[0][s]);
                        MFMA32(x1[mt][1], aw, g[1][s]);
                    }
                }
            }
            if (TAPE) tape_store<1>(a.c1, row0, a.N, lane, h, x1);
            layer64(A, A_C2, lds + OFF_B_C2, lane, h, x1, x2);
            if (TAPE) tape_store<1>(a.c2, row0, a.N, lane, h, x2);
            const float *w3 = lds + OFF_W3;
            const float o0 = combine_halves(out_dot<0>(w3, h, x2)) + w3[192], o1 = combine_halves(out_dot<0>(w3 + 64, h, x2)) + w3[193],
                        o2 = combine_halves(out_dot<0>(w3 + 128, h, x2)) + w3[194];
            const float cr = TAPE ? sigmoidf(o0) : fast_sigmoid(o0), cg = TAPE ? sigmoidf(o1) : fast_sigmoid(o1),
                        cb = TAPE ? sigmoidf(o2) : fast_sigmoid(o2);
            if (live) {
                a.rgb[ic * 3 + 0] = cr;
                a.rgb[ic * 3 + 1] = cg;
                a.rgb[ic * 3 + 2] = cb;
            }
        }
        {
            f32x16 x1[2][2], x2[2][2];
            layer_geo(A, A_T1, lds + OFF_B_T1, lane, h, g, x1);
            if (TAPE) tape_store<1>(a.t1, row0, a.N, lane, h, x1);
            layer64(A, A_T2, lds + OFF_B_T2, lane, h, x1, x2);
            if (TAPE) {
                tape_store<2>(a.t2, row0, a.N, lane, h, x2);
            } else {
#pragma unroll
                for (int mt = 0; mt < 2; ++mt) {
#pragma unroll
                    for (int nt = 0; nt < 2; ++nt) {
#pragma unroll
                        for (int r = 0; r < 16; ++r) x2[mt][nt][r] = fast_sigmoid(x2[mt][nt][r]);
                    }
                }
            }
            const float *wt = lds + OFF_WTH;
            float p0 = 0.0f, p1 = 0.0f;
#pragma unroll
            for (int mt = 0; mt < 2; ++mt) {
#pragma unroll
                for (int q = 0; q < 4; ++q) {
                    const float4 w = *reinterpret_cast<const float4 *>(wt + 32 * mt + 8 * q + 4 * h);
                    const float ww[4] = {w.x, w.y, w.z, w.w};
#pragma unroll
                    for (int e = 0; e < 4; ++e) {
                        p0 = fmaf(ww[e], x2[mt][0][4 * q + e], p0);
                        p1 = fmaf(ww[e], x2[mt][1][4 * q + e], p1);
                    }
                }
            }
            const float th = combine_halves(make_float2(p0, p1)) + wt[64];
            if (live) a.thermal[ic] = th;
        }
    }
}

inline bool mfma_supported(const tn_thermal_field *f) {
    return f && f->geo_feat_dim == GF && f->app_dim == APP && f->grid.num_levels == L16;
}

}

namespace tn {

int launch_main_mfma(const tn_thermal_field *field, const tn_render_config *cfg, const tn_render_inputs *in,
                     const tn_render_outputs *out, long long num_rays, const float *spacing_ws, DepthSlots minmax,
                     hipStream_t stream, int split, float *seg_scratch) {
    if (!mfma_supported(field) || !field->prepared) return TN_ERR_UNSUPPORTED;
    MfmaArgs a;
    a.g = tn_make_grid(field->grid);
    a.space = field->space;
    a.blob = field->prepared;
    a.appearance = field->appearance;
    a.avg = field->average_init_density;
    a.sh_shifted = field->sh_shifted;
    a.origins = in->origins; a.dirs = in->directions; a.nears = in->nears; a.fars = in->fars;
    a.cam = in->camera_indices;
    a.spacing = spacing_ws;
    a.R = num_rays; a.S = cfg->num_nerf_samples; a.training = cfg->training; a.lin = cfg->initial_sampler == 1;
    a.rgb = out->rgb; a.acc = out->accumulation; a.depth = out->depth; a.expected = out->expected_depth;
    a.thermal = out->thermal; a.out_w = out->weights[2]; a.minmax = minmax;
    a.early_eps = cfg->training ? 0.0f : fminf(fmaxf(cfg->early_stop_transmittance, 0.0f), 0.25f);
    a.split = 1; a.seg_len = a.S; a.seg_rec = nullptr; a.seg_cum = nullptr;
    const size_t smem = (size_t)LDS_FLOATS * sizeof(float);
    const long long cap = 256LL * 2;
    const size_t smem_rays = (size_t)RAYS_LDS_FLOATS * sizeof(float);
    const long long cap_rays = 256;
    const bool small_call = tn_render_kernel_form(field, cfg, num_rays, 1) == 2;
    if (!cfg->training && !out->weights[2] && !small_call) {
        const bool dense = a.g.num_dense >= kFieldDense;
        if (split > 1 && seg_scratch && a.early_eps == 0.0f) {
            const long long groups = (num_rays + 63) / 64;
            a.seg_len = (a.S + split - 1) / split;
            a.split = (a.S + a.seg_len - 1) / a.seg_len;
            a.seg_rec = seg_scratch;
            a.seg_cum = seg_scratch + (size_t)groups * a.split * SEG_ROWS * 64;
            if (!(dense ? tn_ensure_dynamic_lds<main_mfma_rays_kernel<true, true>>(smem_rays)
                        : tn_ensure_dynamic_lds<main_mfma_rays_kernel<false, true>>(smem_rays)))
                return TN_ERR_LAUNCH;
            const long long need = (groups * a.split + kRaysWaves - 1) / kRaysWaves;
            const unsigned grid = (unsigned)(need < cap_rays ? (need < 1 ? 1 : need) : cap_rays);
            if (dense)
                hipLaunchKernelGGL((main_mfma_rays_kernel<true, true>), dim3(grid), dim3(kRaysBlock), smem_rays, stream, a);
            else
                hipLaunchKernelGGL((main_mfma_rays_kernel<false, true>), dim3(grid), dim3(kRaysBlock), smem_rays, stream, a);
            hipLaunchKernelGGL(segments_combine_kernel, dim3((unsigned)((num_rays + 255) / 256)), dim3(256), 0, stream, a);
            if (hipGetLastError() != hipSuccess) return TN_ERR_LAUNCH;
            return TN_OK;
        }
        a.split = 1;
        if (!(dense ? tn_ensure_dynamic_lds<main_mfma_rays_kernel<true>>(smem_rays) : tn_ensure_dynamic_lds<main_mfma_rays_kernel<false>>(smem_rays)))
            return TN_ERR_LAUNCH;
        const long long groups = (num_rays + 63) / 64;
        const long long need = (groups + kRaysWaves - 1) / kRaysWaves;
        const unsigned grid = (unsigned)(need < cap_rays ? (need < 1 ? 1 : need) : cap_rays);
        if (dense)
            hipLaunchKernelGGL(main_mfma_rays_kernel<true>, dim3(grid), dim3(kRaysBlock), smem_rays, stream, a);
        else
            hipLaunchKernelGGL(main_mfma_rays_kernel<false>, dim3(grid), dim3(kRaysBlock), smem_rays, stream, a);
        if (hipGetLastError() != hipSuccess) return TN_ERR_LAUNCH;
        return TN_OK;
    }
    if (!tn_ensure_dynamic_lds<main_mfma_kernel>(smem)) return TN_ERR_LAUNCH;
    const long long need = (num_rays + kWaves - 1) / kWaves;
    const unsigned grid = (unsigned)(need < cap ? (need < 1 ? 1 : need) : cap);
    hipLaunchKernelGGL(main_mfma_kernel, dim3(grid), dim3(kBlock), smem, stream, a);
    if (hipGetLastError() != hipSuccess) return TN_ERR_LAUNCH;
    return TN_OK;
}

}

extern "C" {
#if TN_FIELD_STAMPS
int tn_field_stamps_read(unsigned int *dst, size_t count) {
    if (hipDeviceSynchronize() != hipSuccess) return TN_ERR_LAUNCH;
    return hipMemcpyFromSymbol(dst, HIP_SYMBOL(tn_field_stamp_buf), count * sizeof(unsigned int)) == hipSuccess ? TN_OK : TN_ERR_LAUNCH;
}
#endif

int tn_field_fwd_taped(const tn_thermal_field *f, const float *positions, const float *directions,
                       const int32_t *camera_indices, int64_t num_rays, int32_t n, float *enc, float *selector, float *h1,
                       float *bo, float *density, float *c1, float *c2, float *rgb, float *t1, float *t2, float *thermal,
                       void *stream) {
    if (num_rays == 0) return TN_OK;
    if (!f || !positions || !directions || !camera_indices) return TN_ERR_NULL;
    if (!enc || !selector || !h1 || !bo || !density || !c1 || !c2 || !rgb || !t1 || !t2 || !thermal) return TN_ERR_NULL;
    if (num_rays < 0 || n < 1) return TN_ERR_SHAPE;
    TN_TRY(tn_check_thermal_field(f));
    if (!mfma_supported(f) || !f->prepared) return TN_ERR_UNSUPPORTED;
    TapedArgs a;
    a.g = tn_make_grid(f->grid);
    a.space = f->space;
    a.blob = f->prepared;
    a.appearance = f->appearance;
    a.avg = f->average_init_density;
    a.sh_shifted = f->sh_shifted;
    a.positions = positions; a.dirs = directions; a.cam = camera_indices;
    a.N = (long long)num_rays * n; a.n = n;
    a.enc = enc; a.sel = selector; a.h1 = h1; a.bo = bo; a.density = density; a.c1 = c1; a.c2 = c2; a.rgb = rgb;
    a.t1 = t1; a.t2 = t2; a.thermal = thermal; a.ray_bias = nullptr; a.jac = nullptr;
    const size_t smem = (size_t)LDS_FLOATS * sizeof(float);
    if (!tn_ensure_dynamic_lds<field_fwd_taped_kernel<true>>(smem)) return TN_ERR_LAUNCH;
    const long long passes = (a.N + 63) / 64;
    const long long need = (passes + kWaves - 1) / kWaves;
    const unsigned grid = (unsigned)(need < 512 ? (need < 1 ? 1 : need) : 512);
    hipLaunchKernelGGL(field_fwd_taped_kernel<true>, dim3(grid), dim3(kBlock), smem, (hipStream_t)stream, a);
    if (hipGetLastError() != hipSuccess) return TN_ERR_LAUNCH;
    return TN_OK;
}

int tn_field_fwd_train(const tn_thermal_field *f, const float *positions, const float *ray_bias, int64_t num_rays, int32_t n,
                       float *enc, float *selector, float *density, float *rgb, float *thermal, float *base_out, float *position_jacobian,
                       void *stream) {
    if (num_rays == 0) return TN_OK;
    if (!f || !positions || !ray_bias || !enc || !selector || !density || !rgb || !thermal) return TN_ERR_NULL;
    if (num_rays < 0 || n < 1) return TN_ERR_SHAPE;
    TN_TRY(tn_check_thermal_field(f));
    if (!mfma_supported(f) || !f->prepared) return TN_ERR_UNSUPPORTED;
    TapedArgs a;
    a.g = tn_make_grid(f->grid);
    a.space = f->space;
    a.blob = f->prepared;
    a.appearance = f->appearance;
    a.avg = f->average_init_density;
    a.sh_shifted = f->sh_shifted;
    a.positions = positions; a.dirs = nullptr; a.cam = nullptr;
    a.N = (long long)num_rays * n; a.n = n;
    a.enc = enc; a.sel = selector; a.h1 = nullptr; a.bo = base_out; a.density = density; a.c1 = nullptr; a.c2 = nullptr; a.rgb = rgb;
    a.t1 = nullptr; a.t2 = nullptr; a.thermal = thermal; a.ray_bias = ray_bias; a.jac = position_jacobian;
    const size_t smem = (size_t)LDS_FLOATS * sizeof(float);
    if (!tn_ensure_dynamic_lds<field_fwd_taped_kernel<false>>(smem) || !tn_ensure_dynamic_lds<field_fwd_taped_kernel<false, true>>(smem))
        return TN_ERR_LAUNCH;
    const long long passes = (a.N + 63) / 64;
    const long long need = (passes + kWaves - 1) / kWaves;
    const unsigned grid = (unsigned)(need < 512 ? (need < 1 ? 1 : need) : 512);
    if (a.jac) hipLaunchKernelGGL((field_fwd_taped_kernel<false, true>), dim3(grid), dim3(kBlock), smem, (hipStream_t)stream, a);
    else hipLaunchKernelGGL(field_fwd_taped_kernel<false>, dim3(grid), dim3(kBlock), smem, (hipStream_t)stream, a);
// ... 28 lines not shown
```

### thermo_nerf_amd/engine.py

```python
from __future__ import annotations

from typing import Dict, List, Optional, Tuple

import torch
from torch import Tensor

from . import _hip
from .samplers import linspace_bins, pdf_positions
from .nerfacto_config.thermal_nerfacto import KERNEL_FAMILY
from .thermal_nerf.thermal_nerf_model import ThermalNerfModel

OUTPUT_KEYS = ("rgb", "accumulation", "depth", "expected_depth", "prop_depth_0", "prop_depth_1", "thermal")


class RayRenderEngine:
    def __init__(self, model: ThermalNerfModel, chunk: Optional[int] = None, streams: Optional[int] = None,
                 fuse_chunks: bool = True, max_workspace_bytes: int = 2 << 30) -> None:
        if model.training:
            raise RuntimeError("RayRenderEngine renders in eval mode; call model.eval() first")
        if getattr(model.field, "staged", False):
            raise RuntimeError("RayRenderEngine drives the fused kernels (64-wide MLP layers); this field is staged (other widths): "
                               "render it through model.get_outputs_for_camera_ray_bundle")
        self.model = model
        self.chunk = int(chunk or model.config.eval_num_rays_per_chunk)
        self.lib = _hip.load()
        cfg = model.config
        self.P0, self.P1 = cfg.num_proposal_samples_per_ray
        self.S = cfg.num_nerf_samples_per_ray
        self.rc = _hip.tn_render_config()
        self.rc.num_proposal_samples[0], self.rc.num_proposal_samples[1] = self.P0, self.P1
        self.rc.num_nerf_samples = self.S
        self.rc.training = 0
        self.rc.pdf_anneal = float(model.proposal_sampler._anneal)
        self.rc.early_stop_transmittance = float(cfg.early_termination_eps)
        self.rc.kernel_family = 0
        self.rc.initial_sampler = int(model.proposal_sampler.initial_sampler.uniform_spacing)
        self.fuse_chunks = bool(fuse_chunks) and self.chunk % 64 == 0
        if streams is None:
            streams = 2 if (self.fuse_chunks or self.chunk >= 32768) else 4
        self.num_streams = max(1, int(streams))
        self._chunks_whole = self._chunks_slot = 1
        if self.fuse_chunks:
            per_chunk = max(self.lib.tn_render_workspace_bytes(self.rc, self.chunk), 1)
            self._chunks_whole = max(1, int(max_workspace_bytes) // per_chunk)
            self._chunks_slot = max(1, int(max_workspace_bytes) // self.num_streams // per_chunk)
        self.launch_rays = self._chunks_slot * self.chunk
        self._streams: List[torch.cuda.Stream] = []
        self._ws: Optional[Tensor] = None
        self._ws_rays = 0
        self._nf: Optional[Tuple[Tensor, Tensor]] = None
        self._nf_key = None
        self.timings: List[Tuple[torch.cuda.Event, torch.cuda.Event, torch.cuda.Event]] = []

    def _buffers(self, dev, rays_per_launch: Optional[int] = None, launches: int = 2) -> None:
        rays = int(rays_per_launch or self.launch_rays)
        need = self.lib.tn_render_workspace_bytes(self.rc, rays)
        need = (need + 255) // 256 * 256
        slots = min(self.num_streams, max(launches, 1))
        if self._ws is None or self._ws.shape[1] < need or self._ws.shape[0] < slots or self._ws.device != dev:
            self._ws = None
            self._ws = torch.empty((slots, need), dtype=torch.uint8, device=dev)
        if slots > 1 and (len(self._streams) < self.num_streams or self._streams[0].device != self._ws.device):
            self._streams = _hip.concurrent_streams(dev, self.num_streams, with_main=False)
        self._ws_rays = max(self._ws_rays, rays)
        col = self.model.collider
        near = float(col.near_plane if not col.reset_near_plane else 0.0)
        if self._nf is not None and self._nf[0].shape[0] >= rays and self._nf_key == (near, float(col.far_plane), str(dev)):
            return
        self._nf = (torch.full((rays,), near, dtype=torch.float32, device=dev),
                    torch.full((rays,), float(col.far_plane), dtype=torch.float32, device=dev))
        self._nf_key = (near, float(col.far_plane), str(dev))

    def allocate_outputs(self, n: int, dev) -> Dict[str, Tensor]:
        out = {"rgb": torch.empty((n, 3), dtype=torch.float32, device=dev)}
        for k in OUTPUT_KEYS[1:]:
            out[k] = torch.empty((n, 1), dtype=torch.float32, device=dev)
        return out

    def _inputs(self, dev):
        ins = _hip.tn_render_inputs()
        ins.camera_indices = None
        ins.jitter = None
        ins.lin_bins0 = linspace_bins(self.P0, dev).data_ptr()
        ins.u1 = pdf_positions(self.P1 + 1, dev, False).data_ptr()
        ins.u2 = pdf_positions(self.S + 1, dev, False).data_ptr()
        return ins

    def frame_launch_rays(self, frame_rays: int) -> int:
        n_chunks = -(-max(int(frame_rays), 1) // self.chunk)
        if n_chunks <= self._chunks_whole:
            return n_chunks * self.chunk
        k = -(-n_chunks // self._chunks_slot)
        return -(-n_chunks // k) * self.chunk

    def _launch_pieces(self, start: int, end: int, frame_rays: int) -> List[Tuple[int, int]]:
        L = self.frame_launch_rays(frame_rays)
        return [(max(start, k * L), min(end, (k + 1) * L)) for k in range(start // L, (end - 1) // L + 1)] if end > start else []

    def _forms(self, fld, frame_rays: int, piece_start: int, sample_split: Optional[int] = None) -> Tuple[int, int, int]:
        L = self.frame_launch_rays(frame_rays)
        family = KERNEL_FAMILY[self.model.config.kernel_family]
        k = piece_start // L
        whole = min((k + 1) * L, frame_rays) - k * L
        request = self._split_request(sample_split)
        saved = self.rc.kernel_family, self.rc.sample_split
        try:
            self.rc.sample_split = request
            if family == 0 and self.num_streams > 1 and frame_rays > L and L >= 49152:
                prop = field = 1
            else:
                self.rc.kernel_family = family
                prop, field = (int(self.lib.tn_render_kernel_form(None, self.rc, whole, 0)),
                               int(self.lib.tn_render_kernel_form(fld, self.rc, whole, 1)))
            self.rc.kernel_family = field
            split = int(self.lib.tn_render_sample_split(fld, self.rc, frame_rays))
        finally:
            self.rc.kernel_family, self.rc.sample_split = saved
        return prop, field, split

    def _split_request(self, sample_split: Optional[int]) -> int:
        if sample_split is None:
            sample_split = int(getattr(self.model.config, "sample_split", 0) or 0)
            return max(sample_split, 0)
        return max(int(sample_split), 1)

    @torch.no_grad()
    def render(self, origins: Tensor, directions: Tensor, out: Optional[Dict[str, Tensor]] = None,
               record_events: bool = False, nears: Optional[Tensor] = None, fars: Optional[Tensor] = None,
               sample_split: Optional[int] = None) -> Dict[str, Tensor]:
        o = _hip.require_device_tensor(origins, "origins")
        d = _hip.require_device_tensor(directions, "directions")
        n, dev = o.shape[0], o.device
        pieces = self._launch_pieces(0, n, n)
        self._buffers(dev, max((j - i for i, j in pieces), default=1), len(pieces))
        if out is None:
            out = self.allocate_outputs(n, dev)
        prop0, prop1, fld = self.model._c_structs()
        ins = self._inputs(dev)
        if (nears is None) != (fars is None):
            raise ValueError("pass both nears and fars, or neither")
        if nears is not None:
            nears = _hip.require_device_tensor(nears.reshape(-1), "nears")
            fars = _hip.require_device_tensor(fars.reshape(-1), "fars")
            if nears.shape[0] != n or fars.shape[0] != n:
                raise ValueError("nears/fars must hold one value per ray")
        outs = _hip.tn_render_outputs()
        wsn = self._ws.shape[1]
        multi = self.num_streams > 1 and len(pieces) > 1
        family = KERNEL_FAMILY[self.model.config.kernel_family]
        chunked = self.fuse_chunks and n > self.chunk
        bounds = torch.empty((-(-n // self.chunk), 2), dtype=torch.float32, device=dev) if chunked else None
        current = torch.cuda.current_stream(dev)
        if multi:
            for st in self._streams:
                st.wait_stream(current)
        for ci, (i, j) in enumerate(pieces):
            r = j - i
            slot = ci % self.num_streams if multi else 0
            st = self._streams[slot] if multi else current
            stream = st.cuda_stream
            ws = self._ws[slot].data_ptr()
            ins.origins, ins.directions = o.data_ptr() + 12 * i, d.data_ptr() + 12 * i
            if nears is not None:
                ins.nears, ins.fars = nears.data_ptr() + 4 * i, fars.data_ptr() + 4 * i
            else:
                ins.nears, ins.fars = self._nf[0].data_ptr(), self._nf[1].data_ptr()
            outs.rgb = out["rgb"].data_ptr() + 12 * i
            for k in OUTPUT_KEYS[1:]:
                setattr(outs, k, out[k].data_ptr() + 4 * i)
            if record_events:
                e0, e1, e2 = (torch.cuda.Event(enable_timing=True) for _ in range(3))
                e0.record(st)
            form_prop, form_field, split = self._forms(fld, n, i, sample_split)
            self.rc.kernel_family, self.rc.sample_split = form_prop, split
            _hip.check(self.lib.tn_proposal_sample_fwd(prop0, prop1, self.rc, ins, outs, r, ws, wsn, stream),
                       "tn_proposal_sample_fwd")
            if record_events:
                e1.record(st)
            self.rc.kernel_family = form_field
            if chunked:
                _hip.check(self.lib.tn_field_render_chunked_fwd(fld, self.rc, ins, outs, r, ws, wsn, i, self.chunk,
                                                                bounds.data_ptr() + 8 * (i // self.chunk), 1, stream),
                           "tn_field_render_chunked_fwd")
            else:
                _hip.check(self.lib.tn_field_render_fwd(fld, self.rc, ins, outs, r, ws, wsn, stream), "tn_field_render_fwd")
            if record_events:
                e2.record(st)
                self.timings.append((e0, e1, e2))
        self.rc.kernel_family, self.rc.sample_split = family, 0
        if multi:
            for st in self._streams:
                current.wait_stream(st)
        return out

    @torch.no_grad()
    def render_shard(self, origins: Tensor, directions: Tensor, start: int, frame_rays: int,
                     out: Optional[Dict[str, Tensor]] = None, nears: Optional[Tensor] = None,
                     fars: Optional[Tensor] = None, sample_split: Optional[int] = None) -> Tuple[Dict[str, Tensor], Tensor]:
        if not self.fuse_chunks:
            raise RuntimeError("render_shard needs fuse_chunks (a chunk size that is a multiple of 64 rays)")
        o = _hip.require_device_tensor(origins, "origins")
        d = _hip.require_device_tensor(directions, "directions")
        n, dev = o.shape[0], o.device
        if out is None:
            out = self.allocate_outputs(n, dev)
        bounds = torch.empty((-(-frame_rays // self.chunk), 2), dtype=torch.float32, device=dev)
        bounds[:, 0] = float("inf")
        bounds[:, 1] = float("-inf")
        if n == 0:
            return out, bounds
        if start < 0 or start + n > frame_rays or start % 64 != 0:
            raise ValueError("a shard lies inside the frame and starts on a multiple of 64 rays")
        if (nears is None) != (fars is None):
            raise ValueError("pass both nears and fars, or neither")
        if nears is not None:
            nears = _hip.require_device_tensor(nears.reshape(-1), "nears")
            fars = _hip.require_device_tensor(fars.reshape(-1), "fars")
            if nears.shape[0] != n or fars.shape[0] != n:
                raise ValueError("nears/fars must hold one value per ray of the shard")
        pieces = self._launch_pieces(start, start + n, frame_rays)
        self._buffers(dev, max((j - i for i, j in pieces), default=1), len(pieces))
        prop0, prop1, fld = self.model._c_structs()
        ins = self._inputs(dev)
        ins.nears, ins.fars = self._nf[0].data_ptr(), self._nf[1].data_ptr()
        outs = _hip.tn_render_outputs()
        wsn = self._ws.shape[1]
        family = KERNEL_FAMILY[self.model.config.kernel_family]
        current = torch.cuda.current_stream(dev)
        multi = self.num_streams > 1 and len(pieces) > 1
        if multi:
            for st in self._streams:
                st.wait_stream(current)
        for ci, (p0, p1) in enumerate(pieces):
            i, r = p0 - start, p1 - p0
            slot = ci % self.num_streams if multi else 0
            st = self._streams[slot] if multi else current
            ws = self._ws[slot].data_ptr()
            ins.origins, ins.directions = o.data_ptr() + 12 * i, d.data_ptr() + 12 * i
            if nears is not None:
                ins.nears, ins.fars = nears.data_ptr() + 4 * i, fars.data_ptr() + 4 * i
            outs.rgb = out["rgb"].data_ptr() + 12 * i
            for k in OUTPUT_KEYS[1:]:
                setattr(outs, k, out[k].data_ptr() + 4 * i)
            fam_prop, fam_field, split = self._forms(fld, frame_rays, p0, sample_split)
            self.rc.kernel_family, self.rc.sample_split = fam_prop, split
            _hip.check(self.lib.tn_proposal_sample_fwd(prop0, prop1, self.rc, ins, outs, r, ws, wsn, st.cuda_stream),
                       "tn_proposal_sample_fwd")
            self.rc.kernel_family = fam_field
            _hip.check(self.lib.tn_field_render_chunked_fwd(fld, self.rc, ins, outs, r, ws, wsn, p0, self.chunk,
                                                            bounds.data_ptr() + 8 * (p0 // self.chunk), 0, st.cuda_stream),
                       "tn_field_render_chunked_fwd")
        self.rc.kernel_family, self.rc.sample_split = family, 0
        if multi:
            for st in self._streams:
                current.wait_stream(st)
        return out, bounds

    def shard_sample_split(self, shard_rays: int) -> int:
        _, _, fld = self.model._c_structs()
        saved = self.rc.kernel_family, self.rc.sample_split
        self.rc.kernel_family, self.rc.sample_split = 1, 0
        k = int(self.lib.tn_render_sample_split(fld, self.rc, max(int(shard_rays), 1)))
        self.rc.kernel_family, self.rc.sample_split = saved
        return k

    def apply_depth_bounds(self, out: Dict[str, Tensor], start: int, bounds: Tensor) -> None:
        b = _hip.require_device_tensor(bounds, "bounds")
        n = out["expected_depth"].shape[0]
        _hip.check(self.lib.tn_expected_depth_clip_chunked(out["expected_depth"].data_ptr(), n, start, self.chunk,
                                                           b.data_ptr() + 8 * (start // self.chunk), _hip.current_stream()),
                   "tn_expected_depth_clip_chunked")

    def drain_timings(self) -> Tuple[List[float], List[float]]:
        prop = [a.elapsed_time(b) for a, b, _ in self.timings]
        main = [b.elapsed_time(c) for _, b, c in self.timings]
        self.timings = []
        return prop, main


def engine_for(model, cached: Optional[RayRenderEngine]) -> RayRenderEngine:
    chunk = int(model.config.eval_num_rays_per_chunk)
    eng = cached
    if eng is None or eng.chunk != chunk or eng.rc.early_stop_transmittance != float(model.config.early_termination_eps):
        eng = RayRenderEngine(model, chunk=chunk)
    eng.rc.pdf_anneal = float(model.proposal_sampler._anneal)
    return eng
```

### thermo_nerf_amd/nerfacto_config/thermal_nerfacto.py

```python
from __future__ import annotations

from dataclasses import dataclass, field
from typing import Any, Dict, List, Literal, Tuple, Type, Union

import torch
from torch import Tensor, nn

from ..camera_optimizer import CameraOptimizerConfig
from ..rays import RayBundle
from ..scene import SceneBox


@dataclass
class NerfactoModelConfig:

    _target: Type = field(default_factory=lambda: ThermalNerfactoModel)
    near_plane: float = 0.05
    far_plane: float = 1000.0
    background_color: Literal["random", "last_sample", "black", "white"] = "last_sample"
    hidden_dim: int = 64
    hidden_dim_color: int = 64
    hidden_dim_transient: int = 64
    num_levels: int = 16
    base_res: int = 16
# ... 44 lines not shown
    """>0: the proposal networks' eval kernels read their leading hash levels from a dense re-layout built within this budget
    per network (dense[x][y][z] = (table[hash(x,y,z)], its x-neighbour's entry minus it): bit-identical results; an x pair
    of corners is one aligned 16-byte load and its lerp one fma, so a level costs 4 gather instructions instead of 8).  64 MB holds 5
    and 4 of the reference's 2 x 5 proposal levels (45 + 41 MB); rebuilt when the tables change; never used in training."""
    field_dense_grid_budget_mb: int = 16
    """The same for the main field's 16-level grid: 16 MB holds the 6 levels (14.5 MB) the lane = ray field kernels read
    densely; a smaller budget leaves those kernels on the hashed tables."""
    use_mfma: bool = True
    """Use the MFMA form of the main-field kernel when the library provides it."""
    early_termination_eps: float = 0.0
    """eval only; > 0: a wave of 64 rays stops marching once every ray's transmittance is below this value
    (outputs move by <= eps; 0 = off = the reference's behaviour).  Only the lane = ray kernels (calls of ~60 k rays and
    more) implement it; smaller calls run one ray per wave and render exactly."""
    fused_train_forward: bool = True
    """Training: the final level's field forward (encode + mlp_base + heads, with its tape) as ONE MFMA kernel
    (tn_field_fwd_taped); False: the stage-by-stage entry points (one launch per nerfstudio module)."""
    fused_train_backward: bool = True
    """Training: the backward of each MLP (mlp_head, mlp_thermal + head, mlp_base, the proposal MLPs) as ONE launch per MLP
    (tn_linear_chain_bwd: one tile read per layer); False: one tn_linear_bwd launch per layer."""
    tape_free_training: bool = True
    """Training: the final level's field without an activation tape.  The forward (tn_field_fwd_train) keeps 38 floats per
    sample (hash features, selector, density, rgb, thermal) instead of ~380; the backward (tn_field_bwd_fused) recomputes the
    five hidden layers from the hash features in registers and runs every adjoint next to them (DESIGN §5.6).  False: the
    taped forward + chained / per-layer backward above, kept as the cross-check (same gradients, tests/test_gpu_training.py)."""
    fused_proposal_training: bool = True
    """Training, steps on which the proposal networks take gradient: each level's HashMLPDensityField forward and backward as one
    launch each (tn_density_fwd_train / tn_density_bwd_train: lane = sample, weights as scalars, hidden layer recomputed);
    False: the stage entry points + tn_linear_chain_bwd."""
    fused_backward_split: bool = True
    """tn_field_bwd_fused as three launches (colour head | thermal head | mlp_base) of two waves per SIMD each instead of one
    launch of one wave per SIMD holding all ~210 gradient accumulators (DESIGN §5.6)."""
    trunc_exp_clamp_min: float = -15.0
    """Lower clamp of trunc_exp's backward, g * exp(clamp(x, min, 15)): -15 = nerfstudio's activations.trunc_exp (taken from
    torch-ngp, two-sided); float("-inf") = upper clamp only (SURVEY A.3 [UNSURE])."""
    store_base_output: bool = True
    """Training (round 5, with tape_free_training and fused_backward_split): the forward also keeps mlp_base's 16 output rows
    (64 B per sample, 54 floats per sample in all) and the backward's colour and thermal launches read them instead of
    recomputing mlp_base from the hash features — 48 of a head tile's ~330 MFMAs (DESIGN §5.6)."""
    store_position_jacobian: bool = True
    """Training with ray gradients (camera-pose optimisation; round 5, with tape_free_training and fused_backward_split): the forward
    also writes d hash features / d position (96 floats per sample) while the eight corner values of every level are in its
    registers, and the backward's position gradient is 12 streamed reads per lane instead of 32 table reads (DESIGN §5.6)."""
    backward_bf16_pieces: bool = True
    """Training (round 5, with store_base_output): the 64 x 64 products of the backward's two head launches — the second layer's
    recomputed forward and its dx — on the bf16 matrix cores as six-product splits of three exact bf16 pieces per operand
    (fp32's rounding size per product, the arithmetic of mlp_precision="bf16x6"); the weight-gradient products stay on the fp32
    MFMA (DESIGN §5.6).  False: every product on v_mfma_f32_16x16x4_f32."""
    bucketed_table_scatter: bool = True
    """Training: hash-table gradient of the field's fine levels (scaling >= 200: levels 8-15) as bucketed records + LDS sums instead of
    global atomics (tn_hash_encode_bwd_sorted), the coarse levels with the atomics: 5.03 against 5.25 ms per step at S=192,
    2.24 against 2.27 at S=48 (DESIGN §5.6)."""
    spread_coarse_scatter: bool = True
    """Training: the coarsest levels of the table-gradient scatter (dense vertex grid <= 48^3: the first four levels of the
    reference grids) accumulate into 16 private dense copies that a second launch sums and hashes into the gradient
    (tn_hash_encode_bwd_spread): same-address atomics retire one at a time, and at those levels a trained scene's samples
    share a few thousand entries (DESIGN §5.6)."""
    overlap_table_scatter: bool = True
    """Training: the bucketed part of the field's table-gradient scatter runs on a second HIP stream beside the atomic part —
    disjoint levels of the gradient, one waiting on the memory-side atomic unit, the other on LDS and streaming (DESIGN §5.6)."""
    fused_step_calls: bool = True
    """Training (round 6): on the steps whose proposal networks take no gradient (5 of 6 after warm-up) the forward's launch chain and
    the backward's are ONE C-ABI call each (tn_train_step_fwd / tn_train_step_bwd: the same entry points, order and streams as the
    per-call host path, issued from C++; the step's per-sample tensors in one slab) — ~20 ctypes calls and ~45 allocations per step
    less on the host, which decides the step at the reference's default S = 48.  False: one call per launch (the cross-check)."""
    deferred_table_update: bool = False
    """Training (round 6; set by thermo_nerf_amd.trainer.Trainer with its HipAdam optimizer, off for a foreign training loop): the field's
    table-gradient scatter — both halves — and the table's Adam run on the step's side streams and are NOT joined by the backward:
    the calling stream goes on with everything that needs neither the table nor its gradient (ray-level adjoints, camera-pose
    backward, the small tensors' Adam, the next step's ray gather / camera optimizer / proposal pass / field_prepare) and joins right
    before the next field forward.  Whoever reads ``hash_table`` or its ``.grad`` on another stream in between calls
    ``thermo_nerf_amd._hip.join_pending()`` first (Module.train / state_dict / the eval paths / Trainer.train's exit do)."""
    overlap_regularisers: Union[bool, str] = "auto"
    """Training: the distortion and interlevel terms are launched by the forward itself, on the step's side streams beside
    the depth renderers and the image losses (they depend on the forward's weights and bins only); get_metrics_dict /
    get_loss_dict pick the results up.  False: each is launched where it is asked for; "auto": on from 4096 x 96 final-level
    samples per step, where the step's device time leaves room for the extra stream joins on the host (DESIGN §5.6)."""
    kernel_family: Literal["auto", "lane_ray", "ray_per_wave"] = "auto"
    """Which form of the fused kernels a call runs (tn_render_config.kernel_family): "auto" picks by call size (lane = ray —
    one wave owns 64 consecutive rays — from ~60-80 k rays up, one ray per wave below); the other two force a form."""
    sample_split: int = 0
    """Sample-split tiles of the exact-fp32 lane = ray field kernel (tn_render_config.sample_split): 0 = the library picks the
    number of segments a 64-ray tile's sample march is cut into from the call's size (1 from ~400 k rays up; a 65 536-ray chunk: 2),
    1 = never, k = k segments.  Eval only; same tolerances, other last bits than the serial march (DESIGN §7)."""
    mlp_precision: Literal["f32", "bf16x6", "f16x3"] = "f32"
    """"f32": exact fp32 MFMA (v_mfma_f32_32x32x2_f32).  Eval-only alternatives on the matrix cores' 16-bit rate, fp32 accumulate:
    "bf16x6" — every fp32 operand as three bf16 pieces (24 bits: an exact split), six piece products per fp32 product, 2^-23
    relative per-product error = the size of fp32's own rounding (an fp32 dot product in another order); "f16x3" — two f16
    pieces (22 bits), three products, ~2^-22 (activations must stay below 65504)."""

    def setup(self, **kwargs) -> Any:
        return self._target(self, **kwargs)


@dataclass
class ThermalNerfactoModelConfig(NerfactoModelConfig):

    _target: Type = field(default_factory=lambda: ThermalNerfactoModel)
    max_temperature: float = 1.0
    min_temperature: float = 0.0
    cold: bool = False
    camera_optimizer_mode: Literal["off", "SO3xR3", "SE3"] = "SO3xR3"


KERNEL_FAMILY = {"auto": 0, "lane_ray": 1, "ray_per_wave": 2}


class ThermalNerfactoModel(nn.Module):

    config: ThermalNerfactoModelConfig

    def __init__(self, config: ThermalNerfactoModelConfig, scene_box: SceneBox, num_train_data: int, **kwargs) -> None:
        super().__init__()
        config.camera_optimizer = CameraOptimizerConfig(mode=config.camera_optimizer_mode)
        self.config = config
        self.scene_box = scene_box
        self.num_train_data = num_train_data
        self.kwargs = kwargs
        self.collider = None
        self.max_temperature = config.max_temperature
        self.min_temperature = config.min_temperature
        self.populate_modules()
        self.device_indicator_param = nn.Parameter(torch.empty(0))

    @property
    def device(self):
        return self.device_indicator_param.device

    def populate_modules(self) -> None:
        raise NotImplementedError

    def get_outputs(self, ray_bundle: RayBundle) -> Dict[str, Tensor]:
        raise NotImplementedError

    def forward(self, ray_bundle: RayBundle) -> Dict[str, Tensor]:
        if self.collider is not None:
            ray_bundle = self.collider(ray_bundle)
        return self.get_outputs(ray_bundle)

    @torch.no_grad()
    def get_outputs_for_camera_ray_bundle(self, camera_ray_bundle: RayBundle) -> Dict[str, Tensor]:
        num_rays_per_chunk = self.config.eval_num_rays_per_chunk
        image_height, image_width = camera_ray_bundle.origins.shape[:2]
        num_rays = len(camera_ray_bundle)
        outputs_lists: Dict[str, List[Tensor]] = {}
        for i in range(0, num_rays, num_rays_per_chunk):
            ray_bundle = camera_ray_bundle.get_row_major_sliced_ray_bundle(i, i + num_rays_per_chunk).to(self.device)
            outputs = self.forward(ray_bundle=ray_bundle)
            for name, out in outputs.items():
                if not isinstance(out, Tensor):
                    continue
                outputs_lists.setdefault(name, []).append(out)
        return {k: torch.cat(v).view(image_height, image_width, -1) for k, v in outputs_lists.items()}
```

### thermo_nerf_amd/thermal_nerf/thermal_nerf_model.py

```python
from __future__ import annotations

import weakref
from dataclasses import dataclass, field
from typing import Dict, List, Optional, Sequence, Tuple, Type

import numpy as np
import torch
from torch import Tensor, nn

from .. import _hip
from ..fields import FieldHeadNames, HashMLPDensityField
from ..nerfacto_config.thermal_nerfacto import KERNEL_FAMILY, ThermalNerfactoModel, ThermalNerfactoModelConfig
from ..rays import RayBundle
from ..rendered_image_modalities import RenderedImageModality
from ..renderers import AccumulationRenderer, DepthRenderer, RGBRenderer
from ..samplers import (ProposalNetworkSampler, UniformSampler, draw_jitter, jitter_levels, linspace_bins, pdf_positions,
                        _samples_from_bins)
from ..scene import NearFarCollider, SceneBox, SceneContraction
from .thermal_field import ThermalNerfactoTField
from .thermal_field_head import FieldHeadNamesT
from .thermal_renderer import ThermalRenderer


_ENGINES: "weakref.WeakKeyDictionary" = weakref.WeakKeyDictionary()


@dataclass
class ThermalNerfModelConfig(ThermalNerfactoModelConfig):

    _target: Type = field(default_factory=lambda: ThermalNerfModel)
    use_transient_embedding: bool = False
    thermal_loss_weight: float = 1.0
    pass_thermal_gradients: bool = True


class ThermalNerfModel(ThermalNerfactoModel):
    config: ThermalNerfModelConfig

    def __init__(self, config: ThermalNerfModelConfig, metadata: dict, scene_box: SceneBox, num_train_data: int,
                 **kwargs) -> None:
        if RenderedImageModality.THERMAL.value not in metadata.keys():
            raise ValueError("Thermal images not found in metadata.")
        super().__init__(config, scene_box, num_train_data, **kwargs)
        self.config = config
        self.max_temperature = config.max_temperature
        self.min_temperature = config.min_temperature
        self._workspace: Optional[Tensor] = None
        self._struct_key = None
        self._structs = None

    def populate_modules(self) -> None:
        cfg = self.config
        if cfg.implementation not in ("hip", "tcnn", "torch"):
            raise ValueError(cfg.implementation)
        scene_contraction = None if cfg.disable_scene_contraction else SceneContraction(order=float("inf"))
        budget = int(cfg.dense_grid_budget_mb) << 20

        self.field = ThermalNerfactoTField(
            self.scene_box.aabb, hidden_dim=cfg.hidden_dim, num_levels=cfg.num_levels, max_res=cfg.max_res,
            base_res=cfg.base_res, features_per_level=cfg.features_per_level,
            log2_hashmap_size=cfg.log2_hashmap_size, hidden_dim_color=cfg.hidden_dim_color,
            hidden_dim_transient=cfg.hidden_dim_transient, spatial_distortion=scene_contraction,
            num_images=self.num_train_data, use_pred_normals=cfg.predict_normals,
            use_average_appearance_embedding=cfg.use_average_appearance_embedding,
            appearance_embedding_dim=cfg.appearance_embed_dim, implementation="hip",
            use_transient_embedding=cfg.use_transient_embedding, pass_thermal_gradients=cfg.pass_thermal_gradients,
            sh_input=cfg.sh_input,
        )
        self.field.dense_budget_bytes = int(cfg.field_dense_grid_budget_mb) << 20
        self.camera_optimizer = cfg.camera_optimizer.setup(num_cameras=self.num_train_data, device="cpu")

        self.density_fns = []
        num_prop_nets = cfg.num_proposal_iterations
        self.proposal_networks = nn.ModuleList()
        if cfg.use_same_proposal_network:
            assert len(cfg.proposal_net_args_list) == 1, "Only one proposal network is allowed."
            network = HashMLPDensityField(self.scene_box.aabb, spatial_distortion=scene_contraction,
                                          **cfg.proposal_net_args_list[0], implementation="hip")
            network.dense_budget_bytes = budget
            self.proposal_networks.append(network)
            self.density_fns.extend([network.density_fn for _ in range(num_prop_nets)])
        else:
            for i in range(num_prop_nets):
                args = cfg.proposal_net_args_list[min(i, len(cfg.proposal_net_args_list) - 1)]
                network = HashMLPDensityField(self.scene_box.aabb, spatial_distortion=scene_contraction, **args,
                                              implementation="hip")
                network.dense_budget_bytes = budget
                self.proposal_networks.append(network)
            self.density_fns.extend([network.density_fn for network in self.proposal_networks])

        def update_schedule(step):
            return np.clip(np.interp(step, [0, cfg.proposal_warmup], [0, cfg.proposal_update_every]), 1,
                           cfg.proposal_update_every)

        initial_sampler = None
# ... 183 lines not shown
        ray_samples_list.append(ray_samples)
        rgb = self.renderer_rgb(rgb=field_outputs[FieldHeadNames.RGB], weights=weights)
        depth = self.renderer_depth(weights=weights, ray_samples=ray_samples)
        expected_depth = self.renderer_expected_depth(weights=weights, ray_samples=ray_samples)
        accumulation = self.renderer_accumulation(weights=weights)
        outputs = {
            "rgb": rgb,
            RenderedImageModality.ACCUMULATION.value: accumulation,
            RenderedImageModality.DEPTH.value: depth,
            "expected_depth": expected_depth,
        }
        if self.training:
            outputs["weights_list"] = weights_list
            outputs["ray_samples_list"] = ray_samples_list
        for i in range(self.config.num_proposal_iterations):
            outputs[f"prop_depth_{i}"] = self.renderer_depth(weights=weights_list[i], ray_samples=ray_samples_list[i])
        outputs[RenderedImageModality.THERMAL.value] = self.thermal_renderer(field_outputs[FieldHeadNamesT.THERMAL], weights)
        return outputs

    def train(self, mode: bool = True):
        self.invalidate_prepared()
        _hip.join_pending()
        return super().train(mode)

    def state_dict(self, *args, **kwargs):
        _hip.join_pending()
        return super().state_dict(*args, **kwargs)

    def invalidate_prepared(self) -> None:
        self._struct_key = None
        self.field._prepared_key = None
        mods = self.__dict__.get("_tn_dense_modules")
        if mods is None:
            mods = self.__dict__["_tn_dense_modules"] = [m for m in self.modules() if hasattr(m, "_dense_key")]
        for mod in mods:
            mod._dense_key = None

    def named_parameter_lists(self) -> Tuple[List[str], List[nn.Parameter]]:
        hit = self.__dict__.get("_tn_named_params")
        if hit is None:
            named = list(self.named_parameters())
            hit = self.__dict__["_tn_named_params"] = ([n for n, _ in named], [p for _, p in named])
        return hit

    def _c_structs(self):
        _hip.join_pending()
        key = tuple([(p.data_ptr(), p._version) for p in self.named_parameter_lists()[1]]) + (self.config.use_mfma,
                                                                                              self.config.mlp_precision)
        if self._struct_key != key:
            nets = len(self.proposal_networks)
            self._structs = (self.proposal_networks[0].c_struct(), self.proposal_networks[min(1, nets - 1)].c_struct(),
                             self.field.c_struct(prepare=self.config.use_mfma, precision=self.config.mlp_precision))
            self._struct_key = key
        return self._structs

    def _get_outputs_fused(self, ray_bundle: RayBundle, jitter: Optional[Tensor] = None,
                           want_samples: Optional[bool] = None) -> Dict[str, Tensor]:
        lib = _hip.load()
        cfg = self.config
        training = bool(self.training)
        want_samples = training if want_samples is None else want_samples
        o = _hip.require_device_tensor(ray_bundle.origins, "origins")
        d = _hip.require_device_tensor(ray_bundle.directions, "directions")
        if o.dim() != 2:
            raise ValueError("get_outputs expects a flat ray bundle: origins [R,3]")
        R = o.shape[0]
        dev = o.device
        nears = _hip.require_device_tensor(ray_bundle.nears.reshape(-1), "nears")
        fars = _hip.require_device_tensor(ray_bundle.fars.reshape(-1), "fars")
        P0, P1 = cfg.num_proposal_samples_per_ray
        S = cfg.num_nerf_samples_per_ray
        prop0, prop1, fld = self._c_structs()

        rc = _hip.tn_render_config()
        rc.num_proposal_samples[0], rc.num_proposal_samples[1] = P0, P1
        rc.num_nerf_samples = S
        rc.training = 1 if training else 0
        rc.pdf_anneal = float(self.proposal_sampler._anneal)
        rc.early_stop_transmittance = 0.0 if training else float(cfg.early_termination_eps)
        rc.kernel_family = KERNEL_FAMILY[cfg.kernel_family]
        rc.initial_sampler = int(self.proposal_sampler.initial_sampler.uniform_spacing)
        rc.sample_split = int(getattr(cfg, "sample_split", 0))
        rc.per_sample_jitter = 0 if cfg.use_single_jitter else 1

        ins = _hip.tn_render_inputs()
        ins.origins, ins.directions, ins.nears, ins.fars = o.data_ptr(), d.data_ptr(), nears.data_ptr(), fars.data_ptr()
        cam = None
        if training:
            if ray_bundle.camera_indices is None:
                raise AttributeError("Camera indices are not provided.")
            cam = _hip.require_device_tensor(ray_bundle.camera_indices.reshape(-1).to(torch.int32), "camera_indices",
                                             torch.int32)
            if jitter is None:
                jitter = draw_jitter(R, (P0, P1, S), bool(cfg.use_single_jitter), dev)
            jitter = jitter_levels(jitter, R, (P0, P1, S), bool(cfg.use_single_jitter))[0]
        ins.camera_indices = _hip.ptr(cam)
        ins.jitter = _hip.ptr(jitter) if training else None
        ins.lin_bins0 = linspace_bins(P0, dev).data_ptr()
        ins.u1 = pdf_positions(P1 + 1, dev, training).data_ptr()
        ins.u2 = pdf_positions(S + 1, dev, training).data_ptr()

        buf = torch.empty((9, R), dtype=torch.float32, device=dev)
        rgb = torch.empty((R, 3), dtype=torch.float32, device=dev)
        outs = _hip.tn_render_outputs()
        outs.rgb = rgb.data_ptr()
        names = ["accumulation", "depth", "expected_depth", "prop_depth_0", "prop_depth_1", "thermal"]
        for i, nm in enumerate(names):
            setattr(outs, nm, buf[i].data_ptr())
        extra = {}
        if want_samples:
            ns = (P0, P1, S)
            extra["w"] = [torch.empty((R, n), dtype=torch.float32, device=dev) for n in ns]
            extra["sp"] = [torch.empty((R, n + 1), dtype=torch.float32, device=dev) for n in ns]
            extra["eu"] = [torch.empty((R, n + 1), dtype=torch.float32, device=dev) for n in ns]
            for i in range(3):
                outs.weights[i] = extra["w"][i].data_ptr()
                outs.spacing_bins[i] = extra["sp"][i].data_ptr()
                outs.eucl_bins[i] = extra["eu"][i].data_ptr()

        need = lib.tn_render_workspace_bytes(rc, R)
        if self._workspace is None or self._workspace.numel() < need or self._workspace.device != dev:
            self._workspace = torch.empty(need, dtype=torch.uint8, device=dev)
        _hip.check(
            lib.tn_render_rays_fwd(prop0, prop1, fld, rc, ins, outs, R, self._workspace.data_ptr(),
                                   self._workspace.numel(), _hip.current_stream()),
            "tn_render_rays_fwd",
        )
        outputs: Dict[str, Tensor] = {
            "rgb": rgb,
            RenderedImageModality.ACCUMULATION.value: buf[0][:, None],
            RenderedImageModality.DEPTH.value: buf[1][:, None],
            "expected_depth": buf[2][:, None],
        }
        if want_samples:
            outputs["weights_list"] = [w[..., None] for w in extra["w"]]
            outputs["ray_samples_list"] = [_samples_from_bins(ray_bundle, sp, eu, bool(rc.initial_sampler))
                                           for sp, eu in zip(extra["sp"], extra["eu"])]
        outputs["prop_depth_0"] = buf[3][:, None]
        outputs["prop_depth_1"] = buf[4][:, None]
        outputs[RenderedImageModality.THERMAL.value] = buf[5][:, None]
        return outputs
```

Measured before the change: 20.99 million rays/s.

## Balance last partial tile round by splitting tail tiles into sample segments

Adds a tail-balancing path for the whole-march fp32 field kernel. The last partial round of 64-ray tiles, which leaves wave slots idle, is evaluated as (tile, segment) records over sample ranges and then combined in a replay pass. The segment count is chosen automatically from the tile count and slot count (9 segments for 800x800 at S=192). It costs extra workspace for records and an additional pass, and refactors the per-sample field evaluation into shared device functions.

```diff
diff --git a/include/thermonerf_hip.h b/include/thermonerf_hip.h
--- a/include/thermonerf_hip.h
+++ b/include/thermonerf_hip.h
@@ -212,6 +212,8 @@
     int32_t initial_sampler;
     int32_t sample_split;
     int32_t per_sample_jitter;
+    int32_t tail_balance;
+    int32_t tail_slots;
 } tn_render_config;
 
 typedef struct tn_render_inputs {
@@ -256,6 +258,9 @@
 
 int32_t tn_render_kernel_form(const tn_thermal_field *field, const tn_render_config *cfg, int64_t num_rays, int32_t pass);
 int32_t tn_render_sample_split(const tn_thermal_field *field, const tn_render_config *cfg, int64_t num_rays);
+int32_t tn_render_tail_segments(int64_t tiles, int64_t slots, int32_t num_samples, int32_t request);
+int32_t tn_render_tail_plan(const tn_thermal_field *field, const tn_render_config *cfg, int64_t num_rays);
+size_t tn_render_tail_records_bytes(const tn_render_config *cfg, int64_t num_rays);
 int tn_field_render_chunked_fwd(const tn_thermal_field *field, const tn_render_config *cfg, const tn_render_inputs *in,
                                 const tn_render_outputs *out, int64_t num_rays, void *workspace, size_t workspace_bytes,
                                 int64_t first_ray, int64_t chunk_rays, float *depth_bounds, int32_t clip, void *stream);
diff --git a/thermo_nerf_amd/_hip.py b/thermo_nerf_amd/_hip.py
--- a/thermo_nerf_amd/_hip.py
+++ b/thermo_nerf_amd/_hip.py
@@ -133,6 +133,8 @@
         ("initial_sampler", C.c_int32),
         ("sample_split", C.c_int32),
         ("per_sample_jitter", C.c_int32),
+        ("tail_balance", C.c_int32),
+        ("tail_slots", C.c_int32),
     ]
 
 
@@ -264,6 +266,9 @@
     "tn_depth_bound_slots": (_i64, [_i64, _i64, _i64]),
     "tn_render_kernel_form": (C.c_int32, [C.POINTER(tn_thermal_field), C.POINTER(tn_render_config), _i64, C.c_int32]),
     "tn_render_sample_split": (C.c_int32, [C.POINTER(tn_thermal_field), C.POINTER(tn_render_config), _i64]),
+    "tn_render_tail_segments": (C.c_int32, [_i64, _i64, C.c_int32, C.c_int32]),
+    "tn_render_tail_plan": (C.c_int32, [C.POINTER(tn_thermal_field), C.POINTER(tn_render_config), _i64]),
+    "tn_render_tail_records_bytes": (_sz, [C.POINTER(tn_render_config), _i64]),
     "tn_field_render_chunked_fwd": (
         C.c_int,
         [C.POINTER(tn_thermal_field), C.POINTER(tn_render_config), C.POINTER(tn_render_inputs),
diff --git a/thermo_nerf_amd/csrc/tn_render.hip b/thermo_nerf_amd/csrc/tn_render.hip
--- a/thermo_nerf_amd/csrc/tn_render.hip
+++ b/thermo_nerf_amd/csrc/tn_render.hip
@@ -22,7 +22,7 @@
 namespace tn {
 int launch_main_mfma(const tn_thermal_field *field, const tn_render_config *cfg, const tn_render_inputs *in,
                      const tn_render_outputs *out, long long num_rays, const float *spacing_ws, DepthSlots minmax,
-                     hipStream_t stream, int split, float *seg_scratch);
+                     hipStream_t stream, int split, float *seg_scratch, int tail_k, float *tail_rec, int tail_slots);
 int launch_main_b6(const tn_thermal_field *field, const tn_render_config *cfg, const tn_render_inputs *in,
                    const tn_render_outputs *out, long long num_rays, const float *spacing_ws, DepthSlots minmax,
                    hipStream_t stream);
@@ -786,7 +786,7 @@
 
 extern "C" {
 
-size_t tn_render_workspace_bytes(const tn_render_config *cfg, int64_t num_rays) {
+static size_t render_workspace_base_bytes(const tn_render_config *cfg, int64_t num_rays) {
     if (!cfg || num_rays < 0) return 0;
     const size_t tiles = (size_t)((num_rays + 63) >> 6);
     const int P0 = cfg->num_proposal_samples[0], P1 = cfg->num_proposal_samples[1];
@@ -795,12 +795,18 @@
            tiles * 64 * (nmax + (size_t)P1 + 1) * sizeof(float);
 }
 
+size_t tn_render_workspace_bytes(const tn_render_config *cfg, int64_t num_rays) {
+    if (!cfg || num_rays < 0) return 0;
+    const size_t rec = tn_render_tail_records_bytes(cfg, num_rays);
+    return rec ? align_up(render_workspace_base_bytes(cfg, num_rays), 256) + rec : render_workspace_base_bytes(cfg, num_rays);
+}
+
 static int check_render_common(const tn_render_config *cfg, int64_t num_rays, void *workspace, size_t workspace_bytes) {
     if (!cfg || !workspace) return TN_ERR_NULL;
     const int P0 = cfg->num_proposal_samples[0], P1 = cfg->num_proposal_samples[1], S = cfg->num_nerf_samples;
     if (P0 < 1 || P1 < 1 || S < 1 || P0 > 1024 || P1 > 1024 || S > 1024 || num_rays < 0) return TN_ERR_SHAPE;
     if (cfg->initial_sampler != 0 && cfg->initial_sampler != 1) return TN_ERR_UNSUPPORTED;
-    if (workspace_bytes < tn_render_workspace_bytes(cfg, num_rays)) return TN_ERR_WORKSPACE;
+    if (workspace_bytes < render_workspace_base_bytes(cfg, num_rays)) return TN_ERR_WORKSPACE;
     return TN_OK;
 }
 
@@ -954,7 +960,13 @@
         const int split = out->weights[2] ? 1 : tn_render_sample_split(field, cfg, num_rays);
         float *seg_scratch = reinterpret_cast<float *>(reinterpret_cast<char *>(workspace) +
                                                        align_up(tn_ws_bin_floats(num_rays, S) * sizeof(float), 256) + kWsMid);
-        TN_TRY(launch_main_mfma(field, cfg, in, out, (long long)num_rays, ws_spacing, minmax, s, split, seg_scratch));
+        int tail_k = tn_render_tail_plan(field, cfg, num_rays);
+        const size_t rec_off = align_up(render_workspace_base_bytes(cfg, num_rays), 256);
+        const size_t rec_bytes = tn_render_tail_records_bytes(cfg, num_rays);
+        if (out->weights[2] || rec_bytes == 0 || workspace_bytes < rec_off + rec_bytes) tail_k = 1;
+        float *tail_rec = reinterpret_cast<float *>(reinterpret_cast<char *>(workspace) + rec_off);
+        TN_TRY(launch_main_mfma(field, cfg, in, out, (long long)num_rays, ws_spacing, minmax, s, split, seg_scratch, tail_k, tail_rec,
+                                cfg->tail_slots));
     } else {
         MainArgs ma;
         ma.g = tn_make_grid(field->grid);
@@ -1032,6 +1044,52 @@
     return best;
 }
 
+static inline int64_t tail_slots_of(const tn_render_config *cfg) {
+    return cfg->tail_slots > 0 ? ((int64_t)cfg->tail_slots + 7) / 8 * 8 : 2048;
+}
+
+int32_t tn_render_tail_segments(int64_t tiles, int64_t slots, int32_t num_samples, int32_t request) {
+    constexpr int kMinSeg = 12, kMaxK = 16;
+    if (tiles <= 0 || slots <= 0 || num_samples < 1 || request == 1 || request < 0) return 1;
+    const int64_t rem = tiles % slots;
+    if (tiles < slots || rem == 0) return 1;
+    const int S = num_samples;
+    auto used = [S](int k) { const int len = (S + k - 1) / k; return (S + len - 1) / len; };
+    int kcap = S / kMinSeg;
+    if (kcap > kMaxK) kcap = kMaxK;
+    if (request > 1) {
+        const int k = request < kcap ? request : kcap;
+        return k < 2 ? 1 : used(k);
+    }
+    int best = 1;
+    int64_t best_rounds = 1;
+    for (int k = 2; k <= kcap; ++k) {
+        if (used(k) != k) continue;
+        const int64_t rounds = (rem * k + slots - 1) / slots;
+        if (rounds * best < best_rounds * k) { best = k; best_rounds = rounds; }
+    }
+    return 100 * best_rounds > 95 * best ? 1 : best;
+}
+
+int32_t tn_render_tail_plan(const tn_thermal_field *field, const tn_render_config *cfg, int64_t num_rays) {
+    if (!cfg || num_rays <= 0 || cfg->tail_balance == 1 || cfg->tail_balance < 0) return 1;
+    if (cfg->training || cfg->early_stop_transmittance > 0.0f) return 1;
+    if (field && (!field->prepared || field->prepared_bf16x6 || field->prepared_f16x3)) return 1;
+    tn_thermal_field exact{};
+    if (!field) {
+        exact.prepared = reinterpret_cast<decltype(exact.prepared)>(&exact);
+        field = &exact;
+    }
+    if (tn_render_kernel_form(field, cfg, num_rays, 1) != 1 || tn_render_sample_split(field, cfg, num_rays) != 1) return 1;
+    return tn_render_tail_segments((num_rays + 63) / 64, tail_slots_of(cfg), cfg->num_nerf_samples, cfg->tail_balance);
+}
+
+size_t tn_render_tail_records_bytes(const tn_render_config *cfg, int64_t num_rays) {
+    if (tn_render_tail_plan(nullptr, cfg, num_rays) < 2) return 0;
+    const int64_t tiles = (num_rays + 63) / 64;
+    return (size_t)(tiles % tail_slots_of(cfg)) * (size_t)cfg->num_nerf_samples * 5 * 64 * sizeof(float);
+}
+
 int64_t tn_depth_bound_slots(int64_t first_ray, int64_t num_rays, int64_t chunk_rays) {
     if (num_rays <= 0 || chunk_rays <= 0 || first_ray < 0) return 0;
     return (first_ray + num_rays - 1) / chunk_rays - first_ray / chunk_rays + 1;
diff --git a/thermo_nerf_amd/csrc/tn_render_mfma.hip b/thermo_nerf_amd/csrc/tn_render_mfma.hip
--- a/thermo_nerf_amd/csrc/tn_render_mfma.hip
+++ b/thermo_nerf_amd/csrc/tn_render_mfma.hip
@@ -541,11 +541,9 @@
 #define TN_STAMP(k) do { } while (0)
 #endif
 
-template <bool DENSE, bool SPLIT = false>
-__global__ void __launch_bounds__(kRaysBlock, 1) main_mfma_rays_kernel(MfmaArgs a) {
-    extern __shared__ __attribute__((aligned(16))) float lds[];
+__device__ __forceinline__ void rays_stage_blob(float *lds, const float *blob) {
     {
-        const float4 *src = reinterpret_cast<const float4 *>(a.blob);
+        const float4 *src = reinterpret_cast<const float4 *>(blob);
         float4 *dst = reinterpret_cast<float4 *>(lds);
         for (int i = threadIdx.x; i < RAYS_BLOB_FLOATS / 4; i += kRaysBlock) {
             float4 v = src[i < OFF_W_SH / 4 ? i : i + (OFF_W3 - OFF_W_SH) / 4];
@@ -558,8 +556,143 @@
             dst[i] = v;
         }
     }
+}
+
+__device__ __forceinline__ void rays_tile_bias(const float *lds, int lane, int h, int sh_shifted, float dx, float dy, float dz,
+                                               float4 *c0s, f32x16 &c00) {
+    f32x16 c0[2][2];
+    float sx = dx, sy = dy, sz = dz;
+    if (sh_shifted) {
+        sx = add_rn(sx, 1.0f) / 2.0f; sy = add_rn(sy, 1.0f) / 2.0f; sz = add_rn(sz, 1.0f) / 2.0f;
+    }
+    float c[16];
+    sh16(sx, sy, sz, c);
+#pragma unroll
+    for (int mt = 0; mt < 2; ++mt) {
+        c0[mt][0] = bias_frag(lds + OFF_B_C1_EVAL, mt, h);
+        c0[mt][1] = c0[mt][0];
+    }
+#pragma unroll
+    for (int s = 0; s < 8; ++s) {
+        float bs0, bs1;
+        swap32(c[2 * s], c[2 * s + 1], bs0, bs1);
+#pragma unroll
+        for (int mt = 0; mt < 2; ++mt) {
+            const float aw = lds[OFF_A + (A_SH + mt * 8 + s) * 64 + lane];
+            MFMA32(c0[mt][0], aw, bs0);
+            MFMA32(c0[mt][1], aw, bs1);
+        }
+    }
+    c00 = c0[0][0];
+#pragma unroll
+    for (int q = 0; q < 4; ++q) {
+        c0s[(0 + q) * 64] = make_float4(c0[0][1][4 * q], c0[0][1][4 * q + 1], c0[0][1][4 * q + 2], c0[0][1][4 * q + 3]);
+        c0s[(4 + q) * 64] = make_float4(c0[1][0][4 * q], c0[1][0][4 * q + 1], c0[1][0][4 * q + 2], c0[1][0][4 * q + 3]);
+        c0s[(8 + q) * 64] = make_float4(c0[1][1][4 * q], c0[1][1][4 * q + 1], c0[1][1][4 * q + 2], c0[1][1][4 * q + 3]);
+    }
+}
+
+#if TN_FIELD_STAMPS
+#define TN_STAMP_PARAM , unsigned int (&stamp)[kStampSlots]
+#define TN_STAMP_ARG , stamp
+#else
+#define TN_STAMP_PARAM
+#define TN_STAMP_ARG
+#endif
+template <bool DENSE>
+__device__ __forceinline__ void field_sample(const Grid &g_, const Space &sp, const float *lds, int lane, int h, const float4 *c0s,
+                                             const f32x16 &c00, float ox, float oy, float oz, float dx, float dy, float dz, float s_near,
+                                             float s_far, bool lin, const float *tb, int i, int S, float avg, float &en, float &sb_next,
+                                             float &st, float &step, float &dens, float &cr, float &cg, float &cb,
+                                             float &th TN_STAMP_PARAM) {
+    const float *A = lds + OFF_A;
+    st = en;
+    en = spacing_to_eucl<true>(sb_next, s_near, s_far, lin);
+    sb_next = tb[(size_t)(i + 2 <= S ? i + 2 : S) * 64];
+    step = add_rn(st, en) / 2.0f;
+    float px, py, pz;
+    const float sel = normalize_position<true>(sp, frustum_pos(ox, dx, st, en), frustum_pos(oy, dy, st, en),
+                                         frustum_pos(oz, dz, st, en), px, py, pz);
+    float bt0[16], bt1[16];
+#if TN_FIELD_STAMPS
+    hash_encode_pipelined_raw<L16, LG, DENSE ? kFieldDense : 0, TN_EVAL_GATHER_PRIO>(
+        g_, px, py, pz, [&](int l, const HashTaps &t, const float2 (&fc)[8]) {
+            if (l % LG == 0) TN_STAMP(1 + 2 * (l / LG));
+            const float2 f = hash_blend(t, fc);
+            if (l % LG == 0) TN_STAMP(2 + 2 * (l / LG));
+            swap32(f.x, f.y, bt0[l], bt1[l]);
+        });
+    TN_STAMP(9);
+#else
+    hash_encode_pipelined<L16, LG, DENSE ? kFieldDense : 0, TN_EVAL_GATHER_PRIO>(g_, px, py, pz,
+                                                            [&](int l, float2 f) { swap32(f.x, f.y, bt0[l], bt1[l]); });
+#endif
+#if TN_MFMA_MLP_PRIO
+    __builtin_amdgcn_s_setprio(TN_MFMA_MLP_PRIO);
+#endif
+    f32x16 h1[2][2];
+#pragma unroll
+    for (int mt = 0; mt < 2; ++mt) {
+        h1[mt][0] = bias_frag(lds + OFF_B_BASE1, mt, h);
+        h1[mt][1] = h1[mt][0];
+    }
+#pragma unroll
+    for (int s = 0; s < 16; ++s) {
+#pragma unroll
+        for (int mt = 0; mt < 2; ++mt) {
+            const float aw = A[(A_BASE1 + mt * 16 + s) * 64 + lane];
+            MFMA32(h1[mt][0], aw, bt0[s]);
+            MFMA32(h1[mt][1], aw, bt1[s]);
+        }
+    }
+    float g[2][8];
+    base2_geo<TN_BASE2_STAGED != 0>(A, lds + OFF_B_BASE2, lane, h1, g);
+    float raw, unused;
+    swap32(g[0][0], g[1][0], raw, unused);
+    dens = mul_rn(mul_rn(avg, __expf(raw)), sel);
+    TN_STAMP(10);
+    {
+        f32x16 x1[2][2] = {{c00, c0_frag(c0s)}, {c0_frag(c0s + 4 * 64), c0_frag(c0s + 8 * 64)}}, x2[2][2];
+#pragma unroll
+        for (int s = 0; s < 8; ++s) {
+#pragma unroll
+            for (int mt = 0; mt < 2; ++mt) {
+                const float aw = A[(A_C1 + mt * 8 + s) * 64 + lane];
+                MFMA32(x1[mt][0], aw, g[0][s]);
+                MFMA32(x1[mt][1], aw, g[1][s]);
+            }
+        }
+        layer64(A, A_C2, lds + OFF_B_C2, lane, h, x1, x2);
+        TN_STAMP(11);
+        const float *w3 = lds + RAYS_OFF_W3;
+        cr = fast_sigmoid(combine_halves(out_dot_fast<0>(w3, h, x2)) + w3[192]);
+        cg = fast_sigmoid(combine_halves(out_dot_fast<0>(w3 + 64, h, x2)) + w3[193]);
+        cb = fast_sigmoid(combine_halves(out_dot_fast<0>(w3 + 128, h, x2)) + w3[194]);
+        TN_STAMP(12);
+    }
+#if TN_MFMA_THERMAL_PRIO != TN_MFMA_MLP_PRIO
+    __builtin_amdgcn_s_setprio(TN_MFMA_THERMAL_PRIO);
+#endif
+    {
+        f32x16 x1[2][2], x2[2][2];
+        layer_geo(A, A_T1, lds + OFF_B_T1, lane, h, g, x1);
+        layer64(A, A_T2, lds + OFF_B_T2, lane, h, x1, x2);
+        TN_STAMP(13);
+        const float *wt = lds + RAYS_OFF_WTH;
+        th = combine_halves(out_dot_fast<TN_T2_PRESCALE ? 2 : 1>(wt, h, x2)) + wt[64];
+        TN_STAMP(14);
+    }
+#if TN_MFMA_MLP_PRIO
+    __builtin_amdgcn_s_setprio(0);
+#endif
+    cr = nan_to_num(cr); cg = nan_to_num(cg); cb = nan_to_num(cb); th = nan_to_num(th);
+}
+
+template <bool DENSE, bool SPLIT = false>
+__global__ void __launch_bounds__(kRaysBlock, 1) main_mfma_rays_kernel(MfmaArgs a) {
+    extern __shared__ __attribute__((aligned(16))) float lds[];
+    rays_stage_blob(lds, a.blob);
     __syncthreads();
-    const float *A = lds + OFF_A;
     const Space sp = make_space(a.space);
     const int lane = threadIdx.x & 63, wave = threadIdx.x >> 6, h = lane >> 5;
     const bool lin = a.lin != 0;
@@ -594,38 +727,7 @@
         const float s_near = spacing_fn(a.nears[rc], lin), s_far = spacing_fn(a.fars[rc], lin);
         const float *tb = a.spacing + tn_ws_bin(grp * 64, 0, S) + (rc - grp * 64);
         f32x16 c00;
-        {
-            f32x16 c0[2][2];
-            float sx = dx, sy = dy, sz = dz;
-            if (a.sh_shifted) {
-                sx = add_rn(sx, 1.0f) / 2.0f; sy = add_rn(sy, 1.0f) / 2.0f; sz = add_rn(sz, 1.0f) / 2.0f;
-            }
-            float c[16];
-            sh16(sx, sy, sz, c);
-#pragma unroll
-            for (int mt = 0; mt < 2; ++mt) {
-                c0[mt][0] = bias_frag(lds + OFF_B_C1_EVAL, mt, h);
-                c0[mt][1] = c0[mt][0];
-            }
-#pragma unroll
-            for (int s = 0; s < 8; ++s) {
-                float bs0, bs1;
-                swap32(c[2 * s], c[2 * s + 1], bs0, bs1);
-#pragma unroll
-                for (int mt = 0; mt < 2; ++mt) {
-                    const float aw = A[(A_SH + mt * 8 + s) * 64 + lane];
-                    MFMA32(c0[mt][0], aw, bs0);
-                    MFMA32(c0[mt][1], aw, bs1);
-                }
-            }
-            c00 = c0[0][0];
-#pragma unroll
-            for (int q = 0; q < 4; ++q) {
-                c0s[(0 + q) * 64] = make_float4(c0[0][1][4 * q], c0[0][1][4 * q + 1], c0[0][1][4 * q + 2], c0[0][1][4 * q + 3]);
-                c0s[(4 + q) * 64] = make_float4(c0[1][0][4 * q], c0[1][0][4 * q + 1], c0[1][0][4 * q + 2], c0[1][0][4 * q + 3]);
-                c0s[(8 + q) * 64] = make_float4(c0[1][1][4 * q], c0[1][1][4 * q + 1], c0[1][1][4 * q + 2], c0[1][1][4 * q + 3]);
-            }
-        }
+        rays_tile_bias(lds, lane, h, a.sh_shifted, dx, dy, dz, c0s, c00);
         float en = spacing_to_eucl<true>(tb[(size_t)s0 * 64], s_near, s_far, lin);
         float accum = 0.0f, cum_w = 0.0f;
         float wsum = 0.0f, wr = 0.0f, wg = 0.0f, wbl = 0.0f, wth = 0.0f, wsteps = 0.0f;
@@ -634,86 +736,9 @@
         float sb_next = tb[(size_t)(s0 + 1) * 64];
         for (int i = s0; i < s1; ++i) {
             TN_STAMP(0);
-            const float st = en;
-            en = spacing_to_eucl<true>(sb_next, s_near, s_far, lin);
-            sb_next = tb[(size_t)(i + 2 <= S ? i + 2 : S) * 64];
-            step = add_rn(st, en) / 2.0f;
-            float px, py, pz;
-            const float sel = normalize_position<true>(sp, frustum_pos(ox, dx, st, en), frustum_pos(oy, dy, st, en),
-                                                 frustum_pos(oz, dz, st, en), px, py, pz);
-            float bt0[16], bt1[16];
-#if TN_FIELD_STAMPS
-            hash_encode_pipelined_raw<L16, LG, DENSE ? kFieldDense : 0, TN_EVAL_GATHER_PRIO>(
-                a.g, px, py, pz, [&](int l, const HashTaps &t, const float2 (&fc)[8]) {
-                    if (l % LG == 0) TN_STAMP(1 + 2 * (l / LG));
-                    const float2 f = hash_blend(t, fc);
-                    if (l % LG == 0) TN_STAMP(2 + 2 * (l / LG));
-                    swap32(f.x, f.y, bt0[l], bt1[l]);
-                });
-            TN_STAMP(9);
-#else
-            hash_encode_pipelined<L16, LG, DENSE ? kFieldDense : 0, TN_EVAL_GATHER_PRIO>(a.g, px, py, pz,
-                                                                    [&](int l, float2 f) { swap32(f.x, f.y, bt0[l], bt1[l]); });
-#endif
-#if TN_MFMA_MLP_PRIO
-            __builtin_amdgcn_s_setprio(TN_MFMA_MLP_PRIO);
-#endif
-            f32x16 h1[2][2];
-#pragma unroll
-            for (int mt = 0; mt < 2; ++mt) {
-                h1[mt][0] = bias_frag(lds + OFF_B_BASE1, mt, h);
-                h1[mt][1] = h1[mt][0];
-            }
-#pragma unroll
-            for (int s = 0; s < 16; ++s) {
-#pragma unroll
-                for (int mt = 0; mt < 2; ++mt) {
-                    const float aw = A[(A_BASE1 + mt * 16 + s) * 64 + lane];
-                    MFMA32(h1[mt][0], aw, bt0[s]);
-                    MFMA32(h1[mt][1], aw, bt1[s]);
-                }
-            }
-            float g[2][8];
-            base2_geo<TN_BASE2_STAGED != 0>(A, lds + OFF_B_BASE2, lane, h1, g);
-            float raw, unused;
-            swap32(g[0][0], g[1][0], raw, unused);
-            const float dens = mul_rn(mul_rn(a.avg, __expf(raw)), sel);
-            TN_STAMP(10);
-            {
-                f32x16 x1[2][2] = {{c00, c0_frag(c0s)}, {c0_frag(c0s + 4 * 64), c0_frag(c0s + 8 * 64)}}, x2[2][2];
-#pragma unroll
-                for (int s = 0; s < 8; ++s) {
-#pragma unroll
-                    for (int mt = 0; mt < 2; ++mt) {
-                        const float aw = A[(A_C1 + mt * 8 + s) * 64 + lane];
-                        MFMA32(x1[mt][0], aw, g[0][s]);
-                        MFMA32(x1[mt][1], aw, g[1][s]);
-                    }
-                }
-                layer64(A, A_C2, lds + OFF_B_C2, lane, h, x1, x2);
-                TN_STAMP(11);
-                const float *w3 = lds + RAYS_OFF_W3;
-                cr = fast_sigmoid(combine_halves(out_dot_fast<0>(w3, h, x2)) + w3[192]);
-                cg = fast_sigmoid(combine_halves(out_dot_fast<0>(w3 + 64, h, x2)) + w3[193]);
-                cb = fast_sigmoid(combine_halves(out_dot_fast<0>(w3 + 128, h, x2)) + w3[194]);
-                TN_STAMP(12);
-            }
-#if TN_MFMA_THERMAL_PRIO != TN_MFMA_MLP_PRIO
-            __builtin_amdgcn_s_setprio(TN_MFMA_THERMAL_PRIO);
-#endif
-            {
-                f32x16 x1[2][2], x2[2][2];
-                layer_geo(A, A_T1, lds + OFF_B_T1, lane, h, g, x1);
-                layer64(A, A_T2, lds + OFF_B_T2, lane, h, x1, x2);
-                TN_STAMP(13);
-                const float *wt = lds + RAYS_OFF_WTH;
-                th = combine_halves(out_dot_fast<TN_T2_PRESCALE ? 2 : 1>(wt, h, x2)) + wt[64];
-                TN_STAMP(14);
-            }
-#if TN_MFMA_MLP_PRIO
-            __builtin_amdgcn_s_setprio(0);
-#endif
-            cr = nan_to_num(cr); cg = nan_to_num(cg); cb = nan_to_num(cb); th = nan_to_num(th);
+            float st, dens;
+            field_sample<DENSE>(a.g, sp, lds, lane, h, c0s, c00, ox, oy, oz, dx, dy, dz, s_near, s_far, lin, tb, i, S, a.avg, en, sb_next,
+                                st, step, dens, cr, cg, cb, th TN_STAMP_ARG);
             const float dd = mul_rn(sub_rn(en, st), dens);
             const float wi = nan_to_num(mul_rn(sub_rn(1.0f, __expf(-dd)), __expf(-accum)));
             accum += dd;
@@ -822,6 +847,135 @@
     a.expected[r] = wsteps / add_rn(wsum, 1e-10f);
 }
 
+struct RecordArgs {
+    MfmaArgs m;
+    long long tile0, tiles;
+    int k, seg_len;
+    float *rec;
+};
+constexpr int REC_ROWS = 5;
+
+template <bool DENSE>
+__global__ void __launch_bounds__(kRaysBlock, 1) field_records_kernel(RecordArgs ra) {
+    extern __shared__ __attribute__((aligned(16))) float lds[];
+    const MfmaArgs &a = ra.m;
+    rays_stage_blob(lds, a.blob);
+    __syncthreads();
+    const Space sp = make_space(a.space);
+    const int lane = threadIdx.x & 63, wave = threadIdx.x >> 6, h = lane >> 5;
+    const bool lin = a.lin != 0;
+    const int S = a.S;
+    float4 *c0s = reinterpret_cast<float4 *>(lds + RAYS_OFF_C0) + wave * RAYS_C0_SLOTS * 64 + lane;
+    const long long units = ra.tiles * ra.k;
+    const long long stride = (long long)gridDim.x * kRaysWaves;
+#if TN_FIELD_STAMPS
+    unsigned int stamp[kStampSlots] = {};
+#endif
+    for (long long u = (long long)blockIdx.x * kRaysWaves + wave; u < units; u += stride) {
+        const long long t = u / ra.k;
+        const long long grp = ra.tile0 + t;
+        const int s0 = (int)(u - t * ra.k) * ra.seg_len;
+        const int s1 = s0 + ra.seg_len < S ? s0 + ra.seg_len : S;
+        const long long r = grp * 64 + lane;
+        const long long rc = r < a.R ? r : a.R - 1;
+        const float ox = a.origins[rc * 3], oy = a.origins[rc * 3 + 1], oz = a.origins[rc * 3 + 2];
+        const float dx = a.dirs[rc * 3], dy = a.dirs[rc * 3 + 1], dz = a.dirs[rc * 3 + 2];
+        const float s_near = spacing_fn(a.nears[rc], lin), s_far = spacing_fn(a.fars[rc], lin);
+        const float *tb = a.spacing + tn_ws_bin(grp * 64, 0, S) + (rc - grp * 64);
+        f32x16 c00;
+        rays_tile_bias(lds, lane, h, a.sh_shifted, dx, dy, dz, c0s, c00);
+        float en = spacing_to_eucl<true>(tb[(size_t)s0 * 64], s_near, s_far, lin);
+        float sb_next = tb[(size_t)(s0 + 1) * 64];
+        float *rec = ra.rec + ((size_t)t * S + s0) * (REC_ROWS * 64) + lane;
+        for (int i = s0; i < s1; ++i, rec += REC_ROWS * 64) {
+            float st, step, dens, cr, cg, cb, th;
+            field_sample<DENSE>(a.g, sp, lds, lane, h, c0s, c00, ox, oy, oz, dx, dy, dz, s_near, s_far, lin, tb, i, S, a.avg, en, sb_next,
+                                st, step, dens, cr, cg, cb, th TN_STAMP_ARG);
+            rec[0] = mul_rn(sub_rn(en, st), dens);
+            rec[64] = cr;
+            rec[128] = cg;
+            rec[192] = cb;
+            rec[256] = th;
+        }
+    }
+}
+
+__global__ void __launch_bounds__(256) field_replay_kernel(RecordArgs ra) {
+    const MfmaArgs &a = ra.m;
+    const long long t = (long long)blockIdx.x * 4 + (threadIdx.x >> 6);
+    if (t >= ra.tiles) return;
+    const long long grp = ra.tile0 + t;
+    const int lane = threadIdx.x & 63, S = a.S;
+    const bool lin = a.lin != 0;
+    const long long r = grp * 64 + lane;
+    const bool live = r < a.R;
+    const long long rc = live ? r : a.R - 1;
+    const float s_near = spacing_fn(a.nears[rc], lin), s_far = spacing_fn(a.fars[rc], lin);
+    const float *tb = a.spacing + tn_ws_bin(grp * 64, 0, S) + (rc - grp * 64);
+    const float *rec = ra.rec + (size_t)t * S * (REC_ROWS * 64) + lane;
+    constexpr int PF = 8;
+    float q[PF][REC_ROWS + 1];
+#pragma unroll
+    for (int p = 0; p < PF; ++p) {
+        const int j = p < S ? p : S - 1;
+#pragma unroll
+        for (int k = 0; k < REC_ROWS; ++k) q[p][k] = rec[((size_t)j * REC_ROWS + k) * 64];
+        q[p][REC_ROWS] = tb[(size_t)(j + 1) * 64];
+    }
+    float en = spacing_to_eucl<true>(tb[0], s_near, s_far, lin);
+    float accum = 0.0f, cum_w = 0.0f;
+    float wsum = 0.0f, wr = 0.0f, wg = 0.0f, wbl = 0.0f, wth = 0.0f, wsteps = 0.0f;
+    float cr = 0.0f, cg = 0.0f, cb = 0.0f, th = 0.0f, med = 0.0f, step = 0.0f;
+    float smin = INFINITY, smax = -INFINITY;
+    bool med_found = false;
+    for (int i0 = 0; i0 < S; i0 += PF) {
+#pragma unroll
+        for (int p = 0; p < PF; ++p) {
+            const int i = i0 + p;
+            if (i < S) {
+                const float dd = q[p][0];
+                cr = q[p][1]; cg = q[p][2]; cb = q[p][3]; th = q[p][4];
+                const float st = en;
+                en = spacing_to_eucl<true>(q[p][REC_ROWS], s_near, s_far, lin);
+                const int j = i + PF < S ? i + PF : S - 1;
+#pragma unroll
+                for (int k = 0; k < REC_ROWS; ++k) q[p][k] = rec[((size_t)j * REC_ROWS + k) * 64];
+                q[p][REC_ROWS] = tb[(size_t)(j + 1) * 64];
+                step = add_rn(st, en) / 2.0f;
+                const float wi = nan_to_num(mul_rn(sub_rn(1.0f, __expf(-dd)), __expf(-accum)));
+                accum += dd;
+                cum_w += wi;
+                if (!med_found && cum_w >= 0.5f) {
+                    med_found = true;
+                    med = step;
+                }
+                wsum += wi;
+                wr += mul_rn(wi, cr);
+                wg += mul_rn(wi, cg);
+                wbl += mul_rn(wi, cb);
+                wth += mul_rn(wi, th);
+                wsteps += mul_rn(wi, step);
+                smin = fminf(smin, step);
+                smax = fmaxf(smax, step);
+                if (a.out_w && live) a.out_w[r * S + i] = wi;
+            }
+        }
+    }
+    if (live) {
+        const float bg = sub_rn(1.0f, wsum);
+        const float c0 = add_rn(wr, mul_rn(cr, bg)), c1 = add_rn(wg, mul_rn(cg, bg)), c2 = add_rn(wbl, mul_rn(cb, bg));
+        const float ct = add_rn(wth, mul_rn(th, bg));
+        a.rgb[r * 3 + 0] = fminf(fmaxf(c0, 0.0f), 1.0f);
+        a.rgb[r * 3 + 1] = fminf(fmaxf(c1, 0.0f), 1.0f);
+        a.rgb[r * 3 + 2] = fminf(fmaxf(c2, 0.0f), 1.0f);
+        a.thermal[r] = fminf(fmaxf(ct, 0.0f), 1.0f);
+        a.acc[r] = wsum;
+        a.depth[r] = med_found ? med : step;
+        a.expected[r] = wsteps / add_rn(wsum, 1e-10f);
+    }
+    depth_bounds_flush(a.minmax, a.minmax.slot(grp * 64), smin, smax, lane);
+}
+
 
 struct TapedArgs {
     Grid g;
@@ -1076,7 +1230,7 @@
 
 int launch_main_mfma(const tn_thermal_field *field, const tn_render_config *cfg, const tn_render_inputs *in,
                      const tn_render_outputs *out, long long num_rays, const float *spacing_ws, DepthSlots minmax,
-                     hipStream_t stream, int split, float *seg_scratch) {
+                     hipStream_t stream, int split, float *seg_scratch, int tail_k, float *tail_rec, int tail_slots) {
     if (!mfma_supported(field) || !field->prepared) return TN_ERR_UNSUPPORTED;
     MfmaArgs a;
     a.g = tn_make_grid(field->grid);
@@ -1123,8 +1277,34 @@
         if (!(dense ? tn_ensure_dynamic_lds<main_mfma_rays_kernel<true>>(smem_rays) : tn_ensure_dynamic_lds<main_mfma_rays_kernel<false>>(smem_rays)))
             return TN_ERR_LAUNCH;
         const long long groups = (num_rays + 63) / 64;
+        const long long cap_blocks = tail_slots > 0 ? (tail_slots + kRaysWaves - 1) / kRaysWaves : cap_rays;
+        const long long slots = cap_blocks * kRaysWaves, full = groups / slots * slots, rem = groups - full;
+        if (tail_k > 1 && tail_rec && full > 0 && rem > 0 && a.early_eps == 0.0f) {
+            if (!(dense ? tn_ensure_dynamic_lds<field_records_kernel<true>>(smem_rays) : tn_ensure_dynamic_lds<field_records_kernel<false>>(smem_rays)))
+                return TN_ERR_LAUNCH;
+            RecordArgs ra;
+            ra.m = a;
+            ra.tile0 = full; ra.tiles = rem;
+            ra.seg_len = (a.S + tail_k - 1) / tail_k;
+            ra.k = (a.S + ra.seg_len - 1) / ra.seg_len;
+            ra.rec = tail_rec;
+            MfmaArgs whole = a;
+            whole.R = full * 64;
+            const long long need_rec = (rem * ra.k + kRaysWaves - 1) / kRaysWaves;
+            const unsigned grid_rec = (unsigned)(need_rec < cap_blocks ? need_rec : cap_blocks);
+            if (dense) {
+                hipLaunchKernelGGL(main_mfma_rays_kernel<true>, dim3((unsigned)cap_blocks), dim3(kRaysBlock), smem_rays, stream, whole);
+                hipLaunchKernelGGL(field_records_kernel<true>, dim3(grid_rec), dim3(kRaysBlock), smem_rays, stream, ra);
+            } else {
+                hipLaunchKernelGGL(main_mfma_rays_kernel<false>, dim3((unsigned)cap_blocks), dim3(kRaysBlock), smem_rays, stream, whole);
+                hipLaunchKernelGGL(field_records_kernel<false>, dim3(grid_rec), dim3(kRaysBlock), smem_rays, stream, ra);
+            }
+            hipLaunchKernelGGL(field_replay_kernel, dim3((unsigned)((rem + 3) / 4)), dim3(256), 0, stream, ra);
+            if (hipGetLastError() != hipSuccess) return TN_ERR_LAUNCH;
+            return TN_OK;
+        }
         const long long need = (groups + kRaysWaves - 1) / kRaysWaves;
-        const unsigned grid = (unsigned)(need < cap_rays ? (need < 1 ? 1 : need) : cap_rays);
+        const unsigned grid = (unsigned)(need < cap_blocks ? (need < 1 ? 1 : need) : cap_blocks);
         if (dense)
             hipLaunchKernelGGL(main_mfma_rays_kernel<true>, dim3(grid), dim3(kRaysBlock), smem_rays, stream, a);
         else
diff --git a/thermo_nerf_amd/engine.py b/thermo_nerf_amd/engine.py
--- a/thermo_nerf_amd/engine.py
+++ b/thermo_nerf_amd/engine.py
@@ -7,7 +7,7 @@
 
 from . import _hip
 from .samplers import linspace_bins, pdf_positions
-from .nerfacto_config.thermal_nerfacto import KERNEL_FAMILY
+from .nerfacto_config.thermal_nerfacto import KERNEL_FAMILY, tail_balance_value
 from .thermal_nerf.thermal_nerf_model import ThermalNerfModel
 
 OUTPUT_KEYS = ("rgb", "accumulation", "depth", "expected_depth", "prop_depth_0", "prop_depth_1", "thermal")
@@ -35,13 +35,15 @@
         self.rc.early_stop_transmittance = float(cfg.early_termination_eps)
         self.rc.kernel_family = 0
         self.rc.initial_sampler = int(model.proposal_sampler.initial_sampler.uniform_spacing)
+        self.rc.tail_balance = tail_balance_value(getattr(cfg, "tail_balance", "auto"))
+        self._budget = int(max_workspace_bytes)
         self.fuse_chunks = bool(fuse_chunks) and self.chunk % 64 == 0
         if streams is None:
             streams = 2 if (self.fuse_chunks or self.chunk >= 32768) else 4
         self.num_streams = max(1, int(streams))
         self._chunks_whole = self._chunks_slot = 1
         if self.fuse_chunks:
-            per_chunk = max(self.lib.tn_render_workspace_bytes(self.rc, self.chunk), 1)
+            per_chunk = max(self.lib.tn_render_workspace_bytes(self.rc, self.chunk) - self.lib.tn_render_tail_records_bytes(self.rc, self.chunk), 1)
             self._chunks_whole = max(1, int(max_workspace_bytes) // per_chunk)
             self._chunks_slot = max(1, int(max_workspace_bytes) // self.num_streams // per_chunk)
         self.launch_rays = self._chunks_slot * self.chunk
@@ -52,9 +54,10 @@
         self._nf_key = None
         self.timings: List[Tuple[torch.cuda.Event, torch.cuda.Event, torch.cuda.Event]] = []
 
-    def _buffers(self, dev, rays_per_launch: Optional[int] = None, launches: int = 2) -> None:
+    def _buffers(self, dev, rays_per_launch: Optional[int] = None, launches: int = 2, need: Optional[int] = None) -> None:
         rays = int(rays_per_launch or self.launch_rays)
-        need = self.lib.tn_render_workspace_bytes(self.rc, rays)
+        if need is None:
+            need = self.lib.tn_render_workspace_bytes(self.rc, rays)
         need = (need + 255) // 256 * 256
         slots = min(self.num_streams, max(launches, 1))
         if self._ws is None or self._ws.shape[1] < need or self._ws.shape[0] < slots or self._ws.device != dev:
@@ -118,6 +121,34 @@
             self.rc.kernel_family, self.rc.sample_split = saved
         return prop, field, split
 
+    def _workspace_need(self, fld, pieces, frame_rays: int, sample_split: Optional[int], tail_balance) -> int:
+        saved = self.rc.kernel_family, self.rc.sample_split, self.rc.tail_balance
+        share = self._budget // min(self.num_streams, max(len(pieces), 1))
+        need = 0
+        try:
+            self.rc.tail_balance = self._tail_request(tail_balance)
+            for i, j in pieces:
+                _, self.rc.kernel_family, self.rc.sample_split = self._forms(fld, frame_rays, i, sample_split)
+                whole = int(self.lib.tn_render_workspace_bytes(self.rc, j - i))
+                rec = int(self.lib.tn_render_tail_records_bytes(self.rc, j - i))
+                need = max(need, whole - rec if rec and whole > share else whole)
+        finally:
+            self.rc.kernel_family, self.rc.sample_split, self.rc.tail_balance = saved
+        return need
+
+    def _tail_request(self, tail_balance) -> int:
+        return tail_balance_value(getattr(self.model.config, "tail_balance", "auto") if tail_balance is None else tail_balance)
+
+    def tail_plan(self, rays: int, sample_split: Optional[int] = None, tail_balance=None) -> int:
+        _, _, fld = self.model._c_structs()
+        saved = self.rc.kernel_family, self.rc.sample_split, self.rc.tail_balance
+        try:
+            self.rc.tail_balance = self._tail_request(tail_balance)
+            _, self.rc.kernel_family, self.rc.sample_split = self._forms(fld, rays, 0, sample_split)
+            return int(self.lib.tn_render_tail_plan(fld, self.rc, rays))
+        finally:
+            self.rc.kernel_family, self.rc.sample_split, self.rc.tail_balance = saved
+
     def _split_request(self, sample_split: Optional[int]) -> int:
         if sample_split is None:
             sample_split = int(getattr(self.model.config, "sample_split", 0) or 0)
@@ -127,15 +158,16 @@
     @torch.no_grad()
     def render(self, origins: Tensor, directions: Tensor, out: Optional[Dict[str, Tensor]] = None,
                record_events: bool = False, nears: Optional[Tensor] = None, fars: Optional[Tensor] = None,
-               sample_split: Optional[int] = None) -> Dict[str, Tensor]:
+               sample_split: Optional[int] = None, tail_balance=None) -> Dict[str, Tensor]:
         o = _hip.require_device_tensor(origins, "origins")
         d = _hip.require_device_tensor(directions, "directions")
         n, dev = o.shape[0], o.device
         pieces = self._launch_pieces(0, n, n)
-        self._buffers(dev, max((j - i for i, j in pieces), default=1), len(pieces))
+        prop0, prop1, fld = self.model._c_structs()
+        self._buffers(dev, max((j - i for i, j in pieces), default=1), len(pieces),
+                      need=self._workspace_need(fld, pieces, n, sample_split, tail_balance))
         if out is None:
             out = self.allocate_outputs(n, dev)
-        prop0, prop1, fld = self.model._c_structs()
         ins = self._inputs(dev)
         if (nears is None) != (fars is None):
             raise ValueError("pass both nears and fars, or neither")
@@ -149,6 +181,7 @@
         multi = self.num_streams > 1 and len(pieces) > 1
         family = KERNEL_FAMILY[self.model.config.kernel_family]
         chunked = self.fuse_chunks and n > self.chunk
+        tail_saved, self.rc.tail_balance = self.rc.tail_balance, self._tail_request(tail_balance)
         bounds = torch.empty((-(-n // self.chunk), 2), dtype=torch.float32, device=dev) if chunked else None
         current = torch.cuda.current_stream(dev)
         if multi:
@@ -187,7 +220,7 @@
             if record_events:
                 e2.record(st)
                 self.timings.append((e0, e1, e2))
-        self.rc.kernel_family, self.rc.sample_split = family, 0
+        self.rc.kernel_family, self.rc.sample_split, self.rc.tail_balance = family, 0, tail_saved
         if multi:
             for st in self._streams:
                 current.wait_stream(st)
@@ -196,7 +229,8 @@
     @torch.no_grad()
     def render_shard(self, origins: Tensor, directions: Tensor, start: int, frame_rays: int,
                      out: Optional[Dict[str, Tensor]] = None, nears: Optional[Tensor] = None,
-                     fars: Optional[Tensor] = None, sample_split: Optional[int] = None) -> Tuple[Dict[str, Tensor], Tensor]:
+                     fars: Optional[Tensor] = None, sample_split: Optional[int] = None,
+                     tail_balance=None) -> Tuple[Dict[str, Tensor], Tensor]:
         if not self.fuse_chunks:
             raise RuntimeError("render_shard needs fuse_chunks (a chunk size that is a multiple of 64 rays)")
         o = _hip.require_device_tensor(origins, "origins")
@@ -219,8 +253,10 @@
             if nears.shape[0] != n or fars.shape[0] != n:
                 raise ValueError("nears/fars must hold one value per ray of the shard")
         pieces = self._launch_pieces(start, start + n, frame_rays)
-        self._buffers(dev, max((j - i for i, j in pieces), default=1), len(pieces))
         prop0, prop1, fld = self.model._c_structs()
+        self._buffers(dev, max((j - i for i, j in pieces), default=1), len(pieces),
+                      need=self._workspace_need(fld, pieces, frame_rays, sample_split, tail_balance))
+        tail_saved, self.rc.tail_balance = self.rc.tail_balance, self._tail_request(tail_balance)
         ins = self._inputs(dev)
         ins.nears, ins.fars = self._nf[0].data_ptr(), self._nf[1].data_ptr()
         outs = _hip.tn_render_outputs()
@@ -250,7 +286,7 @@
             _hip.check(self.lib.tn_field_render_chunked_fwd(fld, self.rc, ins, outs, r, ws, wsn, p0, self.chunk,
                                                             bounds.data_ptr() + 8 * (p0 // self.chunk), 0, st.cuda_stream),
                        "tn_field_render_chunked_fwd")
-        self.rc.kernel_family, self.rc.sample_split = family, 0
+        self.rc.kernel_family, self.rc.sample_split, self.rc.tail_balance = family, 0, tail_saved
         if multi:
             for st in self._streams:
                 current.wait_stream(st)
diff --git a/thermo_nerf_amd/nerfacto_config/thermal_nerfacto.py b/thermo_nerf_amd/nerfacto_config/thermal_nerfacto.py
--- a/thermo_nerf_amd/nerfacto_config/thermal_nerfacto.py
+++ b/thermo_nerf_amd/nerfacto_config/thermal_nerfacto.py
@@ -150,6 +150,10 @@
     """Sample-split tiles of the exact-fp32 lane = ray field kernel (tn_render_config.sample_split): 0 = the library picks the
     number of segments a 64-ray tile's sample march is cut into from the call's size (1 from ~400 k rays up; a 65 536-ray chunk: 2),
     1 = never, k = k segments.  Eval only; same tolerances, other last bits than the serial march (DESIGN §7)."""
+    tail_balance: Union[Literal["auto", "off"], int] = "auto"
+    """The last partial round of tiles of a whole-march field call (tn_render_config.tail_balance): "auto" = the library evaluates
+    it as (tile, segment) records plus a replay pass where that fills the wave slots better (tn_render_tail_plan: 9 segments for
+    the 800 x 800 frame at S = 192), "off" = never, k = k segments.  Eval only; the same bits either way (DESIGN §5.2)."""
     mlp_precision: Literal["f32", "bf16x6", "f16x3"] = "f32"
     """"f32": exact fp32 MFMA (v_mfma_f32_32x32x2_f32).  Eval-only alternatives on the matrix cores' 16-bit rate, fp32 accumulate:
     "bf16x6" — every fp32 operand as three bf16 pieces (24 bits: an exact split), six piece products per fp32 product, 2^-23
@@ -171,6 +175,17 @@
 
 
 KERNEL_FAMILY = {"auto": 0, "lane_ray": 1, "ray_per_wave": 2}
+
+
+def tail_balance_value(setting) -> int:
+    if setting in (None, "auto"):
+        return 0
+    if setting == "off":
+        return 1
+    k = int(setting)
+    if k < 2:
+        raise ValueError('tail_balance is "auto", "off" or a number of segments >= 2')
+    return k
 
 
 class ThermalNerfactoModel(nn.Module):
diff --git a/thermo_nerf_amd/thermal_nerf/thermal_nerf_model.py b/thermo_nerf_amd/thermal_nerf/thermal_nerf_model.py
--- a/thermo_nerf_amd/thermal_nerf/thermal_nerf_model.py
+++ b/thermo_nerf_amd/thermal_nerf/thermal_nerf_model.py
@@ -10,7 +10,7 @@
 
 from .. import _hip
 from ..fields import FieldHeadNames, HashMLPDensityField
-from ..nerfacto_config.thermal_nerfacto import KERNEL_FAMILY, ThermalNerfactoModel, ThermalNerfactoModelConfig
+from ..nerfacto_config.thermal_nerfacto import KERNEL_FAMILY, tail_balance_value, ThermalNerfactoModel, ThermalNerfactoModelConfig
 from ..rays import RayBundle
 from ..rendered_image_modalities import RenderedImageModality
 from ..renderers import AccumulationRenderer, DepthRenderer, RGBRenderer
@@ -360,6 +360,7 @@
         rc.initial_sampler = int(self.proposal_sampler.initial_sampler.uniform_spacing)
         rc.sample_split = int(getattr(cfg, "sample_split", 0))
         rc.per_sample_jitter = 0 if cfg.use_single_jitter else 1
+        rc.tail_balance = tail_balance_value(getattr(cfg, "tail_balance", "auto"))
 
         ins = _hip.tn_render_inputs()
         ins.origins, ins.directions, ins.nears, ins.fars = o.data_ptr(), d.data_ptr(), nears.data_ptr(), fars.data_ptr()
```

Result: faster. 21.27 million rays/s (median of 6 runs) (+1.3%).
